# Sharath-girish/Shacira

Measured on AMD Instinct MI355X. Metric: hash-grid samples/sec fwd+bwd (16 lvl, F=2), higher is better.
Workload: dtype f32

## Files before the change

shacira_amd/csrc/api.hip:

```cpp
#include <atomic>
#include <cmath>
#include <cstdint>
#include <cstring>

#include "internal.h"

namespace shacira {

struct OptionSlot {
    const char *name;
    int Options::*field;
    int lo, hi;
    std::atomic<int> value;
};
static OptionSlot g_slots[] = {
    {"fwd_variant", &Options::fwd_variant, -1, 9, {-1}},
    {"bwd_variant", &Options::bwd_variant, -1, 1, {-1}},
    {"mlp_variant", &Options::mlp_variant, -1, 1, {-1}},
    {"bwd_compact", &Options::bwd_compact, 0, 1, {1}},
    {"bwd_selective_zero", &Options::bwd_selective_zero, 0, 1, {1}},
    {"bwd_persistent", &Options::bwd_persistent, 0, 1, {1}},
    {"bwd_fork", &Options::bwd_fork, 0, 1, {1}},
    {"bwd_run_pad", &Options::bwd_run_pad, 0, 1, {1}},
    {"bwd_item12", &Options::bwd_item12, -1, 1, {-1}},
    {"bin_acc_kib", &Options::bin_acc_kib, 0, 128, {0}},
    {"bin_batch_mib", &Options::bin_batch_mib, 1, 1 << 20, {1536}},
    {"tiled", &Options::tiled, -1, 1, {-1}},
    {"tiled_lc_fwd", &Options::tiled_lc_fwd, -1, SHACIRA_MAX_LODS, {-1}},
    {"bwd_brick", &Options::bwd_brick, -1, 1, {-1}},
    {"bwd_brick_lo", &Options::bwd_brick_lo, -1, SHACIRA_MAX_LODS, {-1}},
    {"bwd_brick_hi", &Options::bwd_brick_hi, -1, SHACIRA_MAX_LODS, {-1}},
    {"bwd_brick_fork", &Options::bwd_brick_fork, 0, 2, {2}},
    {"bwd_brick_span", &Options::bwd_brick_span, 0, 64, {0}},
    {"fwd_direct", &Options::fwd_direct, -1, 1, {-1}},
    {"bwd_ext_fork", &Options::bwd_ext_fork, 0, 1, {1}},
    {"coord_variant", &Options::coord_variant, -1, 8, {-1}},
    {"triplane_layout", &Options::triplane_layout, -1, 1, {-1}},
};
static thread_local Options tl_options;
const Options &opt() { return tl_options; }
void options_snapshot() {
    for (OptionSlot &sl : g_slots) tl_options.*(sl.field) = sl.value.load(std::memory_order_relaxed);
}
void options_resolve_item12(int value) { tl_options.bwd_item12 = value; }
static bool option_value_ok(const OptionSlot &sl, int v) {
    if (v < sl.lo || v > sl.hi) return false;
    if (!std::strcmp(sl.name, "fwd_variant")) return v == -1 || v == 0 || v == 3 || v == 6 || v == 8 || v == 9;
    if (!std::strcmp(sl.name, "coord_variant")) return v == -1 || v == 0 || v == 3 || v == 8;
    if (!std::strcmp(sl.name, "bin_acc_kib")) return v == 0 || v == 64 || v == 128;
    return true;
}

static int build_level_table(int dim, int num_lods, int feature_dim, int bw, const int32_t *res_host,
                             int64_t table_rows, LevelTable &lt) {
    if (dim != 2 && dim != 3) return SHACIRA_EINVAL;
    if (num_lods < 1 || num_lods > SHACIRA_MAX_LODS) return SHACIRA_EINVAL;
    if (feature_dim < 1) return SHACIRA_EINVAL;
    if (feature_dim % 2 == 1) return SHACIRA_EODD;
    if (bw < 1 || bw > 30) return SHACIRA_EINVAL;
    if (!res_host || table_rows < 0) return SHACIRA_EINVAL;
    std::memset(&lt, 0, sizeof(lt));
    const int32_t cs = (int32_t)std::pow(2.0, (double)bw);
    for (int l = 0; l < num_lods; ++l) {
        const int32_t r = res_host[l];
        if (r < 1) return SHACIRA_EINVAL;
        lt.res[l] = r;
        lt.hi[l] = (float)((double)r - 1.0 - 1e-5);
        lt.dense[l] = level_is_dense(dim, r, cs) ? 1 : 0;
    }
    lt.mask = (uint32_t)cs - 1u;
    lt.num_lods = num_lods;
    lt.feature_dim = feature_dim;
    lt.table_rows = table_rows;
    lt.level_begin = 0;
    lt.level_end = num_lods;
    lt.stage_flags = 0;
    return 0;
}

}

using namespace shacira;

extern "C" {

int shacira_abi_version(void) { return SHACIRA_ABI_VERSION; }

const char *shacira_strerror(int code) {
    switch (code) {
        case 0: return "success";
        case SHACIRA_EINVAL: return "shacira: invalid argument (dim/sizes/bitwidth/null pointer)";
        case SHACIRA_EDTYPE: return "shacira: unsupported scalar type or operator shape";
        case SHACIRA_EODD: return "The codebook feature dimension needs to be a multiple of 2.";
        case SHACIRA_EWORKSPACE: return "shacira: workspace too small";
        default: break;
    }
    if (code > 0) return hipGetErrorString((hipError_t)code);
    return "shacira: unknown error";
}

int shacira_set_option(const char *name, int value) {
    if (!name) return SHACIRA_EINVAL;
    for (OptionSlot &sl : g_slots) {
        if (std::strcmp(name, sl.name)) continue;
        if (!option_value_ok(sl, value)) return SHACIRA_EINVAL;
        sl.value.store(value, std::memory_order_relaxed);
        return 0;
    }
    return SHACIRA_EINVAL;
}

int shacira_get_option(const char *name) {
    if (!name) return SHACIRA_EINVAL;
    for (OptionSlot &sl : g_slots)
        if (!std::strcmp(name, sl.name)) return sl.value.load(std::memory_order_relaxed);
    return SHACIRA_EINVAL;
}

size_t shacira_hashgrid_forward_workspace_bytes(int dim, int64_t num_coords, int num_lods, int feature_dim,
                                                int codebook_bitwidth, const int32_t *resolutions_host,
                                                int64_t table_rows, int dtype) {
    options_snapshot();
    LevelTable lt;
    if (build_level_table(dim, num_lods, feature_dim, codebook_bitwidth, resolutions_host, table_rows, lt)) return 0;
    return hashgrid_forward_workspace(dim, dtype, lt, num_coords);
}

int shacira_hashgrid_forward(int dim, int64_t num_coords, int num_lods, int feature_dim, int codebook_bitwidth,
                             const int32_t *resolutions_host, const int32_t *codebook_first_idx, int64_t table_rows,
                             const float *coords, const void *codebook, int dtype, void *feats, void *workspace,
                             size_t workspace_bytes, void *stream) {
    return shacira_hashgrid_forward_planned(dim, num_coords, num_lods, feature_dim, codebook_bitwidth, resolutions_host,
                                            codebook_first_idx, table_rows, coords, codebook, dtype, feats, nullptr, 0, 0,
                                            workspace, workspace_bytes, stream);
}

size_t shacira_hashgrid_plan_bytes(int dim, int64_t num_coords, int num_lods, int feature_dim, int codebook_bitwidth,
                                   const int32_t *resolutions_host, int64_t table_rows, int dtype) {
    options_snapshot();
    LevelTable lt;
    if (build_level_table(dim, num_lods, feature_dim, codebook_bitwidth, resolutions_host, table_rows, lt)) return 0;
    if (dtype == SHACIRA_F64 || table_rows == 0 || !tiled_supported(dim, dtype, lt, num_coords)) return 0;
    return sample_plan_bytes(dim, num_coords);
}

int shacira_hashgrid_forward_planned(int dim, int64_t num_coords, int num_lods, int feature_dim, int codebook_bitwidth,
                                     const int32_t *resolutions_host, const int32_t *codebook_first_idx, int64_t table_rows,
                                     const float *coords, const void *codebook, int dtype, void *feats, void *plan,
                                     size_t plan_bytes, int plan_flags, void *workspace, size_t workspace_bytes,
                                     void *stream) {
    options_snapshot();
    LevelTable lt;
    int rc = build_level_table(dim, num_lods, feature_dim, codebook_bitwidth, resolutions_host, table_rows, lt);
    if (rc) return rc;
    if (dtype != SHACIRA_F32 && dtype != SHACIRA_F16 && dtype != SHACIRA_F64) return SHACIRA_EDTYPE;
    if (num_coords < 0) return SHACIRA_EINVAL;
    if (num_coords == 0) return 0;
    if (!codebook_first_idx || !coords || !codebook || !feats) return SHACIRA_EINVAL;
    const size_t need = hashgrid_forward_workspace(dim, dtype, lt, num_coords);
    if (need > 0 && (!workspace || workspace_bytes < need)) return SHACIRA_EWORKSPACE;
    const bool sorts = dtype != SHACIRA_F64 && table_rows > 0 && tiled_supported(dim, dtype, lt, num_coords);
    if (plan != nullptr && sorts && plan_bytes < sample_plan_bytes(dim, num_coords)) return SHACIRA_EWORKSPACE;
    if ((plan_flags & ~SHACIRA_PLAN_READY) != 0 || ((plan_flags & SHACIRA_PLAN_READY) != 0 && plan == nullptr)) return SHACIRA_EINVAL;
    return (int)hashgrid_forward_dispatch(dim, dtype, lt, codebook_first_idx, coords, codebook, feats, workspace,
                                          num_coords, (hipStream_t)stream, sorts ? plan : nullptr,
                                          (plan_flags & SHACIRA_PLAN_READY) != 0);
}

int shacira_hashgrid_debug_corners(int dim, int64_t num_coords, int num_lods, int codebook_bitwidth,
                                   const int32_t *resolutions_host, const float *coords, int32_t *corner_rows,
                                   float *corner_weights, void *stream) {
    LevelTable lt;
    int rc = build_level_table(dim, num_lods, 2, codebook_bitwidth, resolutions_host, 0, lt);
    if (rc) return rc;
    if (num_coords < 0 || num_coords * (int64_t)num_lods >= ((int64_t)1 << 31) * 256) return SHACIRA_EINVAL;
    if (num_coords > 0 && (!coords || (!corner_rows && !corner_weights))) return SHACIRA_EINVAL;
    return (int)hashgrid_debug_corners(dim, lt, coords, num_coords, corner_rows, corner_weights, (hipStream_t)stream);
}

size_t shacira_hashgrid_backward_workspace_bytes(int dim, int64_t num_coords, int num_lods, int feature_dim,
                                                 int codebook_bitwidth, const int32_t *resolutions_host,
                                                 int64_t table_rows, int dtype) {
    options_snapshot();
    LevelTable lt;
    if (build_level_table(dim, num_lods, feature_dim, codebook_bitwidth, resolutions_host, table_rows, lt)) return 0;
    return hashgrid_backward_workspace(dim, dtype, lt, num_coords);
}

int shacira_hashgrid_backward(int dim, int64_t num_coords, int num_lods, int feature_dim, int codebook_bitwidth,
                              const int32_t *resolutions_host, const int32_t *codebook_first_idx, int64_t table_rows,
                              const float *coords, const void *grad_output, int dtype, void *grad_codebook,
                              void *workspace, size_t workspace_bytes, void *stream) {
    return shacira_hashgrid_backward_levels(dim, num_coords, num_lods, feature_dim, codebook_bitwidth, resolutions_host,
                                            codebook_first_idx, table_rows, coords, grad_output, dtype, grad_codebook,
                                            0, num_lods, 0, workspace, workspace_bytes, stream);
}

static int backward_call(int dim, int64_t num_coords, int num_lods, int feature_dim, int codebook_bitwidth,
                         const int32_t *resolutions_host, const int32_t *codebook_first_idx, int64_t table_rows,
                         const float *coords, const void *grad_output, int dtype, void *grad_codebook, int level_begin,
                         int level_end, int flags, const void *plan, size_t plan_bytes, void *workspace,
                         size_t workspace_bytes, void *stream);

size_t shacira_hashgrid_backward_planned_workspace_bytes(int dim, int64_t num_coords, int num_lods, int feature_dim,
                                                         int codebook_bitwidth, const int32_t *resolutions_host,
                                                         int64_t table_rows, int dtype) {
    options_snapshot();
    LevelTable lt;
    if (build_level_table(dim, num_lods, feature_dim, codebook_bitwidth, resolutions_host, table_rows, lt)) return 0;
    LevelTable full = lt;
    const bool sorts = dtype != SHACIRA_F64 && table_rows > 0 && tiled_supported(dim, dtype, full, num_coords);
    if (!sorts) return hashgrid_backward_workspace(dim, dtype, lt, num_coords);
    return hashgrid_backward_workspace_planned(dim, dtype, lt, num_coords, true);
}

int shacira_hashgrid_backward_planned(int dim, int64_t num_coords, int num_lods, int feature_dim, int codebook_bitwidth,
                                      const int32_t *resolutions_host, const int32_t *codebook_first_idx, int64_t table_rows,
                                      const float *coords, const void *grad_output, int dtype, void *grad_codebook,
                                      const void *plan, size_t plan_bytes, void *workspace, size_t workspace_bytes,
                                      void *stream) {
    return backward_call(dim, num_coords, num_lods, feature_dim, codebook_bitwidth, resolutions_host, codebook_first_idx,
                         table_rows, coords, grad_output, dtype, grad_codebook, 0, num_lods, 0, plan, plan_bytes, workspace,
                         workspace_bytes, stream);
}

int shacira_hashgrid_backward_levels(int dim, int64_t num_coords, int num_lods, int feature_dim, int codebook_bitwidth,
                                     const int32_t *resolutions_host, const int32_t *codebook_first_idx,
                                     int64_t table_rows, const float *coords, const void *grad_output, int dtype,
                                     void *grad_codebook, int level_begin, int level_end, int flags, void *workspace,
                                     size_t workspace_bytes, void *stream) {
    return backward_call(dim, num_coords, num_lods, feature_dim, codebook_bitwidth, resolutions_host, codebook_first_idx,
                         table_rows, coords, grad_output, dtype, grad_codebook, level_begin, level_end, flags, nullptr, 0,
                         workspace, workspace_bytes, stream);
}

size_t shacira_hashgrid_coords_backward_workspace_bytes(int dim, int64_t num_coords, int num_lods, int feature_dim,
                                                        int codebook_bitwidth, const int32_t *resolutions_host,
                                                        int64_t table_rows, int dtype) {
    (void)dim; (void)num_coords; (void)num_lods; (void)feature_dim; (void)codebook_bitwidth; (void)resolutions_host;
    (void)table_rows; (void)dtype;
    return 0;
}

int shacira_hashgrid_coords_backward(int dim, int64_t num_coords, int num_lods, int feature_dim, int codebook_bitwidth,
                                     const int32_t *resolutions_host, const int32_t *codebook_first_idx, int64_t table_rows,
                                     const float *coords, const void *codebook, const void *grad_output, int dtype,
                                     float *grad_coords, const void *plan, size_t plan_bytes, void *workspace,
                                     size_t workspace_bytes, void *stream) {
    options_snapshot();
    LevelTable lt;
    int rc = build_level_table(dim, num_lods, feature_dim, codebook_bitwidth, resolutions_host, table_rows, lt);
    if (rc) return rc;
    if (dtype != SHACIRA_F32 && dtype != SHACIRA_F16 && dtype != SHACIRA_F64) return SHACIRA_EDTYPE;
    if (num_coords < 0) return SHACIRA_EINVAL;
    if (num_coords == 0) return 0;
    if (!codebook_first_idx || !coords || !codebook || !grad_output || !grad_coords) return SHACIRA_EINVAL;
    const size_t need = shacira_hashgrid_coords_backward_workspace_bytes(dim, num_coords, num_lods, feature_dim,
                                                                         codebook_bitwidth, resolutions_host, table_rows,
                                                                         dtype);
    if (need > 0 && (!workspace || workspace_bytes < need)) return SHACIRA_EWORKSPACE;
    if (plan != nullptr) {
        const bool sorts = dtype != SHACIRA_F64 && table_rows > 0 && tiled_supported(dim, dtype, lt, num_coords);
        if (!sorts) plan = nullptr;
        else if (plan_bytes < sample_plan_bytes(dim, num_coords)) return SHACIRA_EWORKSPACE;
    }
    return (int)hashgrid_coord_grad_dispatch(dim, dtype, lt, codebook_first_idx, coords, codebook, grad_output, grad_coords,
                                             num_coords, (hipStream_t)stream, plan);
}

size_t shacira_hashgrid_coords_backward2_workspace_bytes(int dim, int64_t num_coords, int num_lods, int feature_dim,
                                                         int codebook_bitwidth, const int32_t *resolutions_host,
                                                         int64_t table_rows, int dtype) {
    LevelTable lt;
    if (build_level_table(dim, num_lods, feature_dim, codebook_bitwidth, resolutions_host, table_rows, lt)) return 0;
    (void)num_coords;
    return dtype == SHACIRA_F16 ? (size_t)table_rows * (size_t)feature_dim * sizeof(float) : 0;
}

int shacira_hashgrid_coords_backward2(int dim, int64_t num_coords, int num_lods, int feature_dim, int codebook_bitwidth,
                                      const int32_t *resolutions_host, const int32_t *codebook_first_idx, int64_t table_rows,
                                      const float *coords, const void *codebook, const void *grad_output,
                                      const float *grad_grad_coords, int dtype, void *grad_grad_output, void *grad_codebook,
                                      float *grad_coords, const void *plan, size_t plan_bytes, void *workspace,
                                      size_t workspace_bytes, void *stream) {
    options_snapshot();
    LevelTable lt;
    int rc = build_level_table(dim, num_lods, feature_dim, codebook_bitwidth, resolutions_host, table_rows, lt);
    if (rc) return rc;
    if (dtype != SHACIRA_F32 && dtype != SHACIRA_F16) return SHACIRA_EDTYPE;
    if (num_coords < 0) return SHACIRA_EINVAL;
    if (!grad_grad_output && !grad_codebook && !grad_coords) return SHACIRA_EINVAL;
    if (num_coords > 0) {
        if (!codebook_first_idx || !coords || !grad_grad_coords) return SHACIRA_EINVAL;
        if (!codebook && (grad_grad_output || grad_coords)) return SHACIRA_EINVAL;
        if (!grad_output && (grad_codebook || grad_coords)) return SHACIRA_EINVAL;
        if (grad_codebook && dtype == SHACIRA_F16 && table_rows > 0) {
            const size_t need = shacira_hashgrid_coords_backward2_workspace_bytes(
                dim, num_coords, num_lods, feature_dim, codebook_bitwidth, resolutions_host, table_rows, dtype);
            if (!workspace || workspace_bytes < need) return SHACIRA_EWORKSPACE;
        }
        if (plan != nullptr) {
            const bool sorts = table_rows > 0 && tiled_supported(dim, dtype, lt, num_coords);
            if (!sorts) plan = nullptr;
            else if (plan_bytes < sample_plan_bytes(dim, num_coords)) return SHACIRA_EWORKSPACE;
        }
    }
    return (int)hashgrid_coord_grad2_dispatch(dim, dtype, lt, codebook_first_idx, coords, codebook, grad_output,
                                              grad_grad_coords, grad_grad_output, grad_codebook, grad_coords, workspace,
                                              num_coords, (hipStream_t)stream, plan);
}

static int triplane_args(int64_t num_coords, int num_lods, const int32_t *lods_host, int feature_dim, TriplaneArgs &a) {
    if (num_coords < 0 || num_coords > (int64_t)INT32_MAX) return SHACIRA_EINVAL;
    if (num_lods < 1 || num_lods > SHACIRA_TRIPLANE_MAX_LODS || !lods_host) return SHACIRA_EINVAL;
    if (feature_dim < 1 || feature_dim > SHACIRA_TRIPLANE_MAX_FDIM) return SHACIRA_EINVAL;
    std::memset(&a, 0, sizeof(a));
    a.num_lods = num_lods;
    a.fdim = feature_dim;
    for (int l = 0; l < num_lods; ++l) {
        if (lods_host[l] < 0 || lods_host[l] > SHACIRA_TRIPLANE_MAX_LOD) return SHACIRA_EINVAL;
        a.side[l] = (1 << lods_host[l]) + 1;
    }
    return 0;
}

static int triplane_pointers(int num_lods, const float *const *host, TriplaneArgs &a, bool grad) {
    if (!host) return SHACIRA_EINVAL;
    for (int q = 0; q < 3 * num_lods; ++q) {
        if (!host[q]) return SHACIRA_EINVAL;
        if (grad) a.grad[q] = const_cast<float *>(host[q]);
        else a.plane[q] = host[q];
    }
    return 0;
}

size_t shacira_triplane_forward_workspace_bytes(int64_t num_coords, int num_lods, const int32_t *lods_host,
                                                int feature_dim, int multiscale_sum) {
    options_snapshot();
    TriplaneArgs a;
    if (triplane_args(num_coords, num_lods, lods_host, feature_dim, a)) return 0;
    return triplane_forward_workspace(a, num_coords);
}

int shacira_triplane_forward(int64_t num_coords, int num_lods, const int32_t *lods_host, int feature_dim,
                             const float *coords, const float *const *planes_host, int multiscale_sum, float *feats,
                             void *workspace, size_t workspace_bytes, void *stream) {
    options_snapshot();
    TriplaneArgs a;
    if (int rc = triplane_args(num_coords, num_lods, lods_host, feature_dim, a)) return rc;
    if (multiscale_sum != 0 && multiscale_sum != 1) return SHACIRA_EINVAL;
    if (num_coords == 0) return 0;
    if (!coords || !feats) return SHACIRA_EINVAL;
    if (int rc = triplane_pointers(num_lods, planes_host, a, false)) return rc;
    const size_t need = triplane_forward_workspace(a, num_coords);
    if (need > 0 && (!workspace || workspace_bytes < need)) return SHACIRA_EWORKSPACE;
    return (int)triplane_forward_dispatch(a, coords, multiscale_sum, feats, workspace, num_coords, (hipStream_t)stream);
}

size_t shacira_triplane_backward_workspace_bytes(int64_t num_coords, int num_lods, const int32_t *lods_host,
                                                 int feature_dim, int multiscale_sum, int flags) {
    TriplaneArgs a;
    if (triplane_args(num_coords, num_lods, lods_host, feature_dim, a)) return 0;
    if ((flags & SHACIRA_TRIPLANE_GRAD_PLANES) == 0) return 0;
    return triplane_backward_workspace(a, multiscale_sum, num_coords);
}

int shacira_triplane_backward(int64_t num_coords, int num_lods, const int32_t *lods_host, int feature_dim,
                              const float *coords, const float *const *planes_host, const float *grad_output,
                              int multiscale_sum, int flags, float *const *grad_planes_host, float *grad_coords,
                              void *workspace, size_t workspace_bytes, void *stream) {
    TriplaneArgs a;
    if (int rc = triplane_args(num_coords, num_lods, lods_host, feature_dim, a)) return rc;
    if (multiscale_sum != 0 && multiscale_sum != 1) return SHACIRA_EINVAL;
    if (flags <= 0 || (flags & ~(SHACIRA_TRIPLANE_GRAD_PLANES | SHACIRA_TRIPLANE_GRAD_COORDS)) != 0) return SHACIRA_EINVAL;
    const bool planes = (flags & SHACIRA_TRIPLANE_GRAD_PLANES) != 0;
    const bool want_coords = (flags & SHACIRA_TRIPLANE_GRAD_COORDS) != 0;
    if (planes)
        if (int rc = triplane_pointers(num_lods, const_cast<const float *const *>(grad_planes_host), a, true)) return rc;
    if (num_coords > 0) {
        if (!coords || !grad_output) return SHACIRA_EINVAL;
        if (want_coords) {
            if (!grad_coords) return SHACIRA_EINVAL;
            if (int rc = triplane_pointers(num_lods, planes_host, a, false)) return rc;
        }
    }
    const size_t need = planes ? triplane_backward_workspace(a, multiscale_sum, num_coords) : 0;
    if (need > 0 && (!workspace || workspace_bytes < need)) return SHACIRA_EWORKSPACE;
    return (int)triplane_backward_dispatch(a, coords, grad_output, multiscale_sum, planes,
                                           want_coords ? grad_coords : nullptr, workspace, num_coords,
                                           (hipStream_t)stream);
}

static int octree_args(int64_t num_coords, int num_levels, const int32_t *levels_host, int feature_dim, OctreeArgs &a) {
    if (num_coords < 0 || num_coords > (int64_t)INT32_MAX) return SHACIRA_EINVAL;
    if (num_levels < 1 || num_levels > SHACIRA_OCTREE_MAX_LEVELS || !levels_host) return SHACIRA_EINVAL;
    if (feature_dim < 1 || feature_dim > SHACIRA_OCTREE_MAX_FDIM) return SHACIRA_EINVAL;
    std::memset(&a, 0, sizeof(a));
    a.num_levels = num_levels;
    a.fdim = feature_dim;
    for (int l = 0; l < num_levels; ++l) {
        if (levels_host[l] < 0 || levels_host[l] > SHACIRA_OCTREE_MAX_LEVEL) return SHACIRA_EINVAL;
        a.level[l] = levels_host[l];
    }
    return 0;
}

static int octree_rows(const int64_t *rows_host, OctreeArgs &a) {
    if (!rows_host) return SHACIRA_EINVAL;
    for (int l = 0; l < a.num_levels; ++l) {
        const int64_t side = ((int64_t)1 << a.level[l]) + 1;
        if (rows_host[l] < 0 || rows_host[l] > side * side * side) return SHACIRA_EINVAL;
        a.rows[l] = rows_host[l];
    }
    return 0;
}

static int octree_index(const void *const *corner_index_host, const void *const *occupancy_host, OctreeArgs &a) {
    if (!corner_index_host || !occupancy_host) return SHACIRA_EINVAL;
    for (int l = 0; l < a.num_levels; ++l) {
        if (!corner_index_host[l] || !occupancy_host[l]) return SHACIRA_EINVAL;
        a.corner[l] = static_cast<const uint2 *>(corner_index_host[l]);
        a.occ[l] = static_cast<const uint32_t *>(occupancy_host[l]);
    }
    return 0;
}

static int octree_tables(const float *const *tables_host, OctreeArgs &a) {
    if (!tables_host) return SHACIRA_EINVAL;
    for (int l = 0; l < a.num_levels; ++l) {
        if (!tables_host[l]) return SHACIRA_EINVAL;
        a.table[l] = tables_host[l];
    }
    return 0;
}

size_t shacira_octree_forward_workspace_bytes(int64_t num_coords, int num_levels, const int32_t *levels_host,
                                              int feature_dim, int multiscale_sum) {
    return 0;
}

int shacira_octree_forward(int64_t num_coords, int num_levels, const int32_t *levels_host, int feature_dim,
                           const float *coords, const float *const *tables_host, const int64_t *rows_host,
                           const void *const *corner_index_host, const void *const *occupancy_host, int multiscale_sum,
                           float *feats, void *workspace, size_t workspace_bytes, void *stream) {
    OctreeArgs a;
    if (int rc = octree_args(num_coords, num_levels, levels_host, feature_dim, a)) return rc;
    if (multiscale_sum != 0 && multiscale_sum != 1) return SHACIRA_EINVAL;
    if (int rc = octree_rows(rows_host, a)) return rc;
    if (num_coords == 0) return 0;
    if (!coords || !feats) return SHACIRA_EINVAL;
    if (int rc = octree_tables(tables_host, a)) return rc;
    if (int rc = octree_index(corner_index_host, occupancy_host, a)) return rc;
    return (int)octree_forward_dispatch(a, coords, multiscale_sum, feats, num_coords, (hipStream_t)stream);
}

size_t shacira_octree_backward_workspace_bytes(int64_t num_coords, int num_levels, const int32_t *levels_host,
                                               int feature_dim, int multiscale_sum, int flags) {
    OctreeArgs a;
    if (octree_args(num_coords, num_levels, levels_host, feature_dim, a)) return 0;
    if ((flags & SHACIRA_OCTREE_GRAD_FEATURES) == 0) return 0;
    return octree_backward_workspace(a, multiscale_sum, num_coords);
}

int shacira_octree_backward(int64_t num_coords, int num_levels, const int32_t *levels_host, int feature_dim,
// ... 800 lines not shown
```

shacira_amd/csrc/hashgrid_fwd.hip:

```cpp
#include <mutex>

#include "hashgrid_rows.h"
#include "internal.h"

namespace shacira {

static bool use_staged(int dim, const LevelTable &lt, int64_t n);
static bool use_lds_tables(int dim, int esz, const LevelTable &lt, int64_t n);

template <typename T, int F> __device__ __forceinline__ void store_row(T *p, const float (&v)[F]) {
    if constexpr (sizeof(T) == 4 && F == 2) {
        *reinterpret_cast<float2 *>(p) = make_float2(v[0], v[1]);
    } else if constexpr (sizeof(T) == 4 && F == 4) {
        *reinterpret_cast<float4 *>(p) = make_float4(v[0], v[1], v[2], v[3]);
    } else if constexpr (sizeof(T) == 2 && F == 2) {
        *reinterpret_cast<__half2 *>(p) = __floats2half2_rn(Scalar<__half>::rounded_fp32(v[0]), Scalar<__half>::rounded_fp32(v[1]));
    } else {
#pragma unroll
        for (int j = 0; j < F; ++j) Scalar<T>::store(p + j, v[j]);
    }
}

template <int DIM, typename T, int F>
__global__ __launch_bounds__(256) void hashgrid_fwd_kernel(LevelTable lt, const int32_t *__restrict__ first_idx,
// ... 530 lines not shown
        int32_t p[DIM];
#pragma unroll
        for (int a = 0; a < DIM; ++a) axis_transform(t[a], res, hi, p[a], f[u][a], g[u][a]);
        const uint32_t ux = (uint32_t)p[0] + (uint32_t)dx;
#pragma unroll
        for (int q = 0; q < NH; ++q) {
            const int dy = (DIM == 3) ? (q >> 1) : q;
            const int dz = (DIM == 3) ? (q & 1) : 0;
            const uint32_t uy = (uint32_t)p[1] + dy;
            uint32_t row;
            if (dense) {
                row = ux + uy * r;
                if constexpr (DIM == 3) row += ((uint32_t)p[2] + dz) * r * r;
            } else {
                row = ux ^ (uy * kPrimeY);
                if constexpr (DIM == 3) row ^= ((uint32_t)p[2] + dz) * kPrimeZ;
                row &= lt.mask;
            }
            const int64_t grow = base + (int64_t)row;
            gather_row<T, F>(table, grow, live[u] && (uint64_t)grow < (uint64_t)lt.table_rows, v[u][q]);
        }
    }
#pragma unroll
    for (int u = 0; u < U; ++u) {
        float pv[NH][F];
#pragma unroll
        for (int q = 0; q < NH; ++q)
#pragma unroll
            for (int j = 0; j < F; ++j)
                pv[q][j] = __builtin_bit_cast(
                    float, __builtin_amdgcn_mov_dpp(__builtin_bit_cast(int, v[u][q][j]), 0xB1, 0xF, 0xF, true));
        if (dx == 0 && live[u]) {
            float acc[F];
#pragma unroll
            for (int k = 0; k < 2 * NH; ++k) {
                const int kx = k / NH, q = k % NH;
                const int dy = (DIM == 3) ? (q >> 1) : q;
                const int dz = (DIM == 3) ? (q & 1) : 0;
                float w = (kx ? f[u][0] : g[u][0]) * (dy ? f[u][1] : g[u][1]);
                if constexpr (DIM == 3) w = w * (dz ? f[u][2] : g[u][2]);
#pragma unroll
                for (int j = 0; j < F; ++j) {
                    const float tv = kx ? pv[q][j] : v[u][q][j];
                    acc[j] = (k == 0) ? tv * w : fmaf(tv, w, acc[j]);
                }
            }
            T *dstT = feats + (int64_t)lvl * level_stride + idx[u] * sample_stride;
            if constexpr (sizeof(T) == 4 && F == 2) {
                typedef float f32x2 __attribute__((ext_vector_type(2)));
                f32x2 o = {acc[0], acc[1]};
                *reinterpret_cast<f32x2 *>(dstT) = o;
            } else {
                store_row<T, F>(dstT, acc);
            }
        }
    }
}

template <typename T, int F>
__global__ __launch_bounds__(256) void untranspose_feats_kernel(const T *__restrict__ src, T *__restrict__ dst,
                                                                int64_t N, int L) {
    struct alignas(sizeof(T) * F) Piece { T v[F]; };
    extern __shared__ __align__(16) unsigned char s_raw_t[];
    Piece *s_tile = reinterpret_cast<Piece *>(s_raw_t);
    const int pitch = L + 1;
    const int64_t s0 = (int64_t)blockIdx.x * 256;
    const int ns = (int)((N - s0 < 256) ? (N - s0) : 256);
    const Piece *in = reinterpret_cast<const Piece *>(src);
    for (int l = 0; l < L; ++l)
        if ((int)threadIdx.x < ns) s_tile[threadIdx.x * pitch + l] = in[(int64_t)l * N + s0 + threadIdx.x];
    __syncthreads();
    const int total = ns * L;
    Piece *out = reinterpret_cast<Piece *>(dst) + s0 * L;
    for (int e = threadIdx.x; e < total; e += 256) {
        const int sm = e / L, l = e - sm * L;
        out[e] = s_tile[sm * pitch + l];
    }
}

template <typename T> static size_t staged_bytes(const LevelTable &lt, int64_t n) {
    return ((size_t)n * lt.num_lods * lt.feature_dim * sizeof(T) + 255) / 256 * 256;
}

template <int DIM, typename T, int F>
static hipError_t launch_fwd(const LevelTable &lt, const int32_t *first_idx, const float *coords, const void *table,
                             void *feats, void *workspace, int64_t num_coords, hipStream_t stream) {
    const int variant = opt().fwd_variant;
    if constexpr (F > 0) {
        if (use_lds_tables(DIM, (int)sizeof(T), lt, num_coords) && ((size_t)lt.num_lods * F * sizeof(T)) % 16 == 0 &&
            (reinterpret_cast<uintptr_t>(feats) & 15u) == 0) {
            LdsFwdPlan plan;
            make_lds_fwd_plan(DIM, lt, sizeof(T), plan);
            static PerDeviceOnce once;
            hipError_t e = once.run([]() -> hipError_t {
                return hipFuncSetAttribute(reinterpret_cast<const void *>(&hashgrid_fwd_lds_kernel<DIM, T, F>),
                                           hipFuncAttributeMaxDynamicSharedMemorySize, (int)kLdsFwdBytes);
            });
            if (e != hipSuccess) return e;
            uint32_t bpg = 256u / (uint32_t)plan.ngroups;
            const uint64_t spw = (uint64_t)kLdsFwdThreads / (uint64_t)plan.P;
            const uint64_t need = ((uint64_t)num_coords + spw - 1) / spw;
            if (bpg > need) bpg = (uint32_t)need;
            if (bpg < 1) bpg = 1;
            hipLaunchKernelGGL((hashgrid_fwd_lds_kernel<DIM, T, F>), dim3(bpg, (uint32_t)plan.ngroups), dim3(kLdsFwdThreads),
                               kLdsFwdBytes, stream, lt, plan, first_idx, coords, static_cast<const T *>(table),
                               static_cast<T *>(feats), num_coords);
            return hipGetLastError();
        }
        if (use_staged(DIM, lt, num_coords) && workspace) {
            const uint32_t tiles = (uint32_t)((num_coords + 128 * kLevelPairU - 1) / (128 * kLevelPairU));
            const uint32_t grid_v6 = 8u * (uint32_t)(((uint64_t)lt.num_lods * tiles + 7) / 8);
            hipError_t e;
            const int d_opt = opt().fwd_direct;
            if (d_opt == 1 || (d_opt < 0 && num_coords <= SHACIRA_FWD_DIRECT_MAX)) {
                hipLaunchKernelGGL((hashgrid_fwd_level_pair_kernel<DIM, T, F>), dim3(grid_v6), dim3(256), 0, stream, lt,
                                   first_idx, coords, static_cast<const T *>(table), static_cast<T *>(feats), num_coords, tiles,
                                   (int64_t)F, (int64_t)lt.num_lods * F);
                return hipGetLastError();
            }
            hipLaunchKernelGGL((hashgrid_fwd_level_pair_kernel<DIM, T, F>), dim3(grid_v6),
                               dim3(256), 0, stream, lt, first_idx, coords, static_cast<const T *>(table),
                               static_cast<T *>(workspace), num_coords, tiles, num_coords * F, (int64_t)F);
            e = hipGetLastError();
            if (e != hipSuccess) return e;
            const size_t shmem = (size_t)256 * (lt.num_lods + 1) * F * sizeof(T);
            static PerDeviceOnce once;
            e = once.run([]() -> hipError_t {
                return hipFuncSetAttribute(reinterpret_cast<const void *>(&untranspose_feats_kernel<T, F>),
                                           hipFuncAttributeMaxDynamicSharedMemorySize, 140 * 1024);
            });
            if (e != hipSuccess) return e;
            hipLaunchKernelGGL((untranspose_feats_kernel<T, F>), dim3((uint32_t)((num_coords + 255) / 256)), dim3(256),
                               shmem, stream, static_cast<const T *>(workspace), static_cast<T *>(feats), num_coords,
                               lt.num_lods);
            return hipGetLastError();
        }
        if (variant == 3 || variant < 0) {
            const uint32_t blocks = (uint32_t)((num_coords + 127) / 128);
            const int LFP = (lt.num_lods * F + 3) / 4 * 4 + 4;
            const size_t shmem = (size_t)128 * LFP * sizeof(float);
            if (shmem <= 64 * 1024) {
                hipLaunchKernelGGL((hashgrid_fwd_pair_kernel<DIM, T, F>), dim3(blocks), dim3(256), shmem, stream, lt,
                                   first_idx, coords, static_cast<const T *>(table), static_cast<T *>(feats),
                                   num_coords);
                return hipGetLastError();
            }
        }
    }
    const int64_t L = lt.num_lods;
    const int64_t max_samples = ((int64_t)1 << 31) / L - 1;
    for (int64_t s0 = 0; s0 < num_coords; s0 += max_samples) {
        const int64_t ns = (num_coords - s0 < max_samples) ? (num_coords - s0) : max_samples;
        const uint32_t items = (uint32_t)(ns * L);
        const uint32_t blocks = (items + 255u) / 256u;
        hipLaunchKernelGGL((hashgrid_fwd_kernel<DIM, T, F>), dim3(blocks), dim3(256), 0, stream, lt, first_idx, coords,
                           static_cast<const T *>(table), static_cast<T *>(feats), s0, items);
        hipError_t e = hipGetLastError();
        if (e != hipSuccess) return e;
    }
    return hipSuccess;
}

template <int DIM, typename T>
static hipError_t dispatch_f(const LevelTable &lt, const int32_t *first_idx, const float *coords, const void *table,
                             void *feats, void *ws, int64_t n, hipStream_t s) {
    switch (lt.feature_dim) {
        case 2: return launch_fwd<DIM, T, 2>(lt, first_idx, coords, table, feats, ws, n, s);
        case 4: return launch_fwd<DIM, T, 4>(lt, first_idx, coords, table, feats, ws, n, s);
        default: return launch_fwd<DIM, T, 0>(lt, first_idx, coords, table, feats, ws, n, s);
    }
}

static bool use_lds_tables(int dim, int esz, const LevelTable &lt, int64_t n) {
    const int v = opt().fwd_variant;
    if (lt.feature_dim != 2 && lt.feature_dim != 4) return false;
    if (v >= 0 && v != 9) return false;
    if (n < 1 || n >= ((int64_t)1 << 31)) return false;
    LdsFwdPlan p;
    if (!make_lds_fwd_plan(dim, lt, (size_t)esz, p)) return false;
    return v == 9 || n >= 4096;
}

static bool use_staged(int dim, const LevelTable &lt, int64_t n) {
    const int v = opt().fwd_variant;
    if (lt.feature_dim != 2 && lt.feature_dim != 4) return false;
    if (v == 6) return true;
    return v < 0 && dim == 3 && n >= 8192;
}

template <int DIM, typename T, int F>
static hipError_t launch_levels_staged(const LevelTable &lt, const int32_t *first_idx, const float *coords,
                                       const void *table, void *staged, int64_t n, hipStream_t s) {
    const uint32_t nl = (uint32_t)(lt.level_end - lt.level_begin);
    const uint32_t tiles = (uint32_t)((n + 128 * kLevelPairU - 1) / (128 * kLevelPairU));
    hipLaunchKernelGGL((hashgrid_fwd_level_pair_kernel<DIM, T, F, true>),
                       dim3(8u * (uint32_t)(((uint64_t)nl * tiles + 7) / 8)), dim3(256), 0, s,
                       lt, first_idx, coords, static_cast<const T *>(table), static_cast<T *>(staged), n, tiles, n * F,
                       (int64_t)F);
    return hipGetLastError();
}

hipError_t hashgrid_forward_levels_staged(int dim, int dtype, const LevelTable &lt, const int32_t *first_idx,
                                          const float *coords, const void *table, void *staged, int64_t n,
                                          hipStream_t s) {
    const int F = lt.feature_dim;
    if (F != 2 && F != 4) return hipErrorInvalidValue;
    if (dim == 3 && dtype == SHACIRA_F32)
        return F == 2 ? launch_levels_staged<3, float, 2>(lt, first_idx, coords, table, staged, n, s)
                      : launch_levels_staged<3, float, 4>(lt, first_idx, coords, table, staged, n, s);
    if (dim == 3)
        return F == 2 ? launch_levels_staged<3, __half, 2>(lt, first_idx, coords, table, staged, n, s)
                      : launch_levels_staged<3, __half, 4>(lt, first_idx, coords, table, staged, n, s);
    if (dtype == SHACIRA_F32)
        return F == 2 ? launch_levels_staged<2, float, 2>(lt, first_idx, coords, table, staged, n, s)
                      : launch_levels_staged<2, float, 4>(lt, first_idx, coords, table, staged, n, s);
    return F == 2 ? launch_levels_staged<2, __half, 2>(lt, first_idx, coords, table, staged, n, s)
                  : launch_levels_staged<2, __half, 4>(lt, first_idx, coords, table, staged, n, s);
}

template <int DIM, typename T, int F>
static hipError_t launch_rows(const LevelTable &lt, const int32_t *first_idx, const float *sorted4,
                              const void *table, const void *staged, void *feats, int64_t n, int lc, hipStream_t s) {
    const uint32_t row_bytes = (uint32_t)(lt.num_lods * F * sizeof(T));
    const size_t shmem = (size_t)128 * ((row_bytes + 15u) / 16u * 16u + 16u);
    static PerDeviceOnce once;
    const hipError_t oe = once.run([]() -> hipError_t {
        return hipFuncSetAttribute(reinterpret_cast<const void *>(&hashgrid_fwd_rows_kernel<DIM, T, F>),
                                   hipFuncAttributeMaxDynamicSharedMemorySize, 140 * 1024);
    });
    if (oe != hipSuccess) return oe;
    const uint32_t blocks = ((uint32_t)((n + 127) / 128) + 7u) & ~7u;
    hipLaunchKernelGGL((hashgrid_fwd_rows_kernel<DIM, T, F>), dim3(blocks), dim3(256), shmem, s, lt,
                       first_idx, reinterpret_cast<const float4 *>(sorted4), static_cast<const T *>(table),
                       static_cast<const T *>(staged), static_cast<T *>(feats), n, lc, 1u);
    return hipGetLastError();
}

hipError_t hashgrid_forward_rows(int dim, int dtype, const LevelTable &lt, const int32_t *first_idx, const float *sorted4,
                                 const void *table, const void *staged, void *feats, int64_t n, int lc, hipStream_t s) {
    const int F = lt.feature_dim;
    if (F != 2 && F != 4) return hipErrorInvalidValue;
    if (dim == 3 && dtype == SHACIRA_F32)
        return F == 2 ? launch_rows<3, float, 2>(lt, first_idx, sorted4, table, staged, feats, n, lc, s)
                      : launch_rows<3, float, 4>(lt, first_idx, sorted4, table, staged, feats, n, lc, s);
    if (dim == 3)
        return F == 2 ? launch_rows<3, __half, 2>(lt, first_idx, sorted4, table, staged, feats, n, lc, s)
                      : launch_rows<3, __half, 4>(lt, first_idx, sorted4, table, staged, feats, n, lc, s);
    if (dtype == SHACIRA_F32)
        return F == 2 ? launch_rows<2, float, 2>(lt, first_idx, sorted4, table, staged, feats, n, lc, s)
                      : launch_rows<2, float, 4>(lt, first_idx, sorted4, table, staged, feats, n, lc, s);
    return F == 2 ? launch_rows<2, __half, 2>(lt, first_idx, sorted4, table, staged, feats, n, lc, s)
                  : launch_rows<2, __half, 4>(lt, first_idx, sorted4, table, staged, feats, n, lc, s);
}

template <int DIM>
__global__ __launch_bounds__(256) void debug_corners_kernel(LevelTable lt, const float *__restrict__ coords, int64_t N,
                                                            int32_t *__restrict__ idx, float *__restrict__ w) {
    constexpr int NC = 1 << DIM;
    const int64_t e = (int64_t)blockIdx.x * 256 + threadIdx.x;
    const int L = lt.num_lods;
    if (e >= N * L) return;
    const int64_t i = e / L;
    const int l = (int)(e - i * L);
    double t[DIM];
#pragma unroll
    for (int a = 0; a < DIM; ++a) t[a] = axis_unit(coords[i * DIM + a]);
    Corners<DIM> c;
    compute_corners<DIM>(t, lt.res[l], lt.hi[l], lt.dense[l] != 0, lt.mask, c);
#pragma unroll
    for (int k = 0; k < NC; ++k) {
        if (idx) idx[e * NC + k] = (int32_t)c.row[k];
        if (w) w[e * NC + k] = c.w[k];
    }
}

hipError_t hashgrid_debug_corners(int dim, const LevelTable &lt, const float *coords, int64_t n, int32_t *idx, float *w,
                                  hipStream_t s) {
    const int64_t items = n * lt.num_lods;
    if (items <= 0) return hipSuccess;
    const uint32_t blocks = (uint32_t)((items + 255) / 256);
    if (dim == 3)
        hipLaunchKernelGGL(debug_corners_kernel<3>, dim3(blocks), dim3(256), 0, s, lt, coords, n, idx, w);
    else
        hipLaunchKernelGGL(debug_corners_kernel<2>, dim3(blocks), dim3(256), 0, s, lt, coords, n, idx, w);
    return hipGetLastError();
}

template <int DIM>
static hipError_t launch_fwd_f64(const LevelTable &lt, const int32_t *first_idx, const float *coords, const void *table,
                                 void *feats, int64_t num_coords, hipStream_t stream) {
    const int64_t L = lt.num_lods;
    const int64_t max_samples = ((int64_t)1 << 31) / L - 1;
    for (int64_t s0 = 0; s0 < num_coords; s0 += max_samples) {
        const int64_t ns = (num_coords - s0 < max_samples) ? (num_coords - s0) : max_samples;
        const uint32_t items = (uint32_t)(ns * L);
        hipLaunchKernelGGL((hashgrid_fwd_kernel<DIM, double, 0>), dim3((items + 255u) / 256u), dim3(256), 0, stream, lt,
                           first_idx, coords, static_cast<const double *>(table), static_cast<double *>(feats), s0, items);
        hipError_t e = hipGetLastError();
        if (e != hipSuccess) return e;
    }
    return hipSuccess;
}

size_t hashgrid_forward_workspace(int dim, int dtype, const LevelTable &lt, int64_t n) {
    if (dtype == SHACIRA_F64) return 0;
    if (tiled_supported(dim, dtype, lt, n)) return tiled_forward_workspace(dim, dtype, lt, n);
    if (lt.feature_dim != 2 && lt.feature_dim != 4) return 0;
    if (use_lds_tables(dim, dtype == SHACIRA_F32 ? 4 : 2, lt, n)) return 0;
    size_t b = ((size_t)n * lt.num_lods * lt.feature_dim * (dtype == SHACIRA_F32 ? 4 : 2) + 255) / 256 * 256;
    return b;
}

hipError_t hashgrid_forward_dispatch(int dim, int dtype, const LevelTable &lt, const int32_t *first_idx,
                                     const float *coords, const void *table, void *feats, void *ws, int64_t n,
                                     hipStream_t s, void *plan, bool plan_ready) {
    if (lt.table_rows == 0) {
        const size_t bytes = (size_t)n * lt.num_lods * lt.feature_dim * (dtype == SHACIRA_F64 ? 8 : dtype == SHACIRA_F32 ? 4 : 2);
        return zero_fill_async(static_cast<float *>(feats), (int64_t)(bytes / 4), s);
    }
    if (dtype == SHACIRA_F64)
        return dim == 3 ? launch_fwd_f64<3>(lt, first_idx, coords, table, feats, n, s)
                        : launch_fwd_f64<2>(lt, first_idx, coords, table, feats, n, s);
    if (tiled_supported(dim, dtype, lt, n)) return tiled_forward(dim, dtype, lt, first_idx, coords, table, feats, ws, n, s, plan, plan_ready);
    if (dim == 3) {
        return dtype == SHACIRA_F32 ? dispatch_f<3, float>(lt, first_idx, coords, table, feats, ws, n, s)
                                    : dispatch_f<3, __half>(lt, first_idx, coords, table, feats, ws, n, s);
    }
    return dtype == SHACIRA_F32 ? dispatch_f<2, float>(lt, first_idx, coords, table, feats, ws, n, s)
                                : dispatch_f<2, __half>(lt, first_idx, coords, table, feats, ws, n, s);
}

}
```

shacira_amd/csrc/hashgrid_tiled.hip:

```cpp
#include <cmath>
#include <mutex>

#include "internal.h"

namespace shacira {

constexpr int kTargetPerBlock = 352;
#ifndef SHACIRA_SORT_TILE
#define SHACIRA_SORT_TILE 4096
#endif
constexpr int kSortTileS = SHACIRA_SORT_TILE;
constexpr int kSortThreadsS = 1024;
constexpr int kMaxBlocksS = 4096;
constexpr int kMaxAxisBlocks = 64;
constexpr uint32_t kCtxMagic = 0x53484354u;

constexpr int kMaxCoarse = 256;
constexpr int kMaxSortTiles = 512;

struct TilePlan {
    int32_t nb[3];
    uint32_t num_blocks;
    int32_t lc;
    uint32_t coarse_shift, num_coarse;
    uint32_t ptiles, chunks_per_tile;
};

struct TileCtx {
    uint32_t *header;
    float4 *sorted4;
    uint32_t *block_start;
    uint32_t *cnt;
    float4 *inter4;
    uint32_t *gcursor;
    uint32_t *cbase;
};

static inline size_t up256(size_t v) { return (v + 255) / 256 * 256; }

__host__ __device__ inline uint32_t axis_block(float c, int nb) {
    const float u = (c + 1.0f) * (0.5f * (float)nb);
    if (!(u < (float)nb)) return (uint32_t)(nb - 1);
    if (!(u >= 0.0f)) return 0u;
    return (uint32_t)(int)u;
}

template <int DIM> __device__ __forceinline__ uint32_t block_key(const float (&c)[DIM], const TilePlan &tp) {
    uint32_t k = axis_block(c[0], tp.nb[0]) + (uint32_t)tp.nb[0] * axis_block(c[1], tp.nb[1]);
    if constexpr (DIM == 3) k += (uint32_t)(tp.nb[0] * tp.nb[1]) * axis_block(c[2], tp.nb[2]);
    return k;
}

static void make_sort_plan(int dim, int64_t n, TilePlan &tp) {
    const double want = (double)n / kTargetPerBlock;
    tp.nb[0] = tp.nb[1] = tp.nb[2] = 1;
    auto clampi = [](double v) { int q = (int)(v + 0.5); return q < 1 ? 1 : (q > kMaxAxisBlocks ? kMaxAxisBlocks : q); };
    if (dim == 3) {
        int m = clampi(std::cbrt(want / 2.0));
        if (m > 12) m = 12;
        tp.nb[0] = tp.nb[1] = m;
        int z = clampi(want / ((double)m * m));
        while ((int64_t)m * m * z > kMaxBlocksS) --z;
        tp.nb[2] = z;
    } else {
        const int m = clampi(std::sqrt(want / 2.0));
        tp.nb[0] = m;
        int y = clampi(want / m);
        while ((int64_t)m * y > kMaxBlocksS) --y;
        tp.nb[1] = y;
    }
    tp.num_blocks = (uint32_t)(tp.nb[0] * tp.nb[1] * tp.nb[2]);
    tp.lc = 0;
    tp.coarse_shift = 0;
    while (((tp.num_blocks + (1u << tp.coarse_shift) - 1) >> tp.coarse_shift) > (uint32_t)kMaxCoarse) ++tp.coarse_shift;
    tp.num_coarse = (tp.num_blocks + (1u << tp.coarse_shift) - 1) >> tp.coarse_shift;
    const int64_t chunks = (n + kSortTileS - 1) / kSortTileS;
    tp.chunks_per_tile = (uint32_t)((chunks + kMaxSortTiles - 1) / kMaxSortTiles);
    if (tp.chunks_per_tile < 1) tp.chunks_per_tile = 1;
    tp.ptiles = (uint32_t)((chunks + tp.chunks_per_tile - 1) / tp.chunks_per_tile);
}

static void make_tile_plan(int dim, const LevelTable &lt, int64_t n, TilePlan &tp) {
    make_sort_plan(dim, n, tp);
    int lc = 0;
    while (lc < lt.num_lods) {
        double cells = 1.0;
        for (int a = 0; a < dim; ++a) cells *= (double)lt.res[lc];
        if (dim == 3 && cells > 32.0 * (double)n) break;
        ++lc;
    }
    const int lc_opt = opt().tiled_lc_fwd;
    if (lc_opt >= 0 && lc_opt <= lt.num_lods) lc = lc_opt;
    tp.lc = lc;
}

static size_t carve_plan(int64_t n, void *buf, TileCtx &c) {
    size_t off = 0;
    auto take = [&](size_t b) { size_t o = off; off = up256(off + b); return o; };
    const size_t o_hdr = take(256);
    const size_t o_sorted = take((size_t)n * sizeof(float4));
    const size_t o_bs = take((size_t)(kMaxBlocksS + 1) * 4);
    unsigned char *p = static_cast<unsigned char *>(buf);
    if (p) {
        c.header = reinterpret_cast<uint32_t *>(p + o_hdr);
        c.sorted4 = reinterpret_cast<float4 *>(p + o_sorted);
        c.block_start = reinterpret_cast<uint32_t *>(p + o_bs);
    }
    return off;
}
static size_t carve_scratch(int dim, int64_t n, void *buf, TileCtx &c) {
    (void)dim;
    size_t off = 0;
    auto take = [&](size_t b) { size_t o = off; off = up256(off + b); return o; };
    const size_t o_cnt = take((size_t)kMaxSortTiles * kMaxCoarse * 4);
    const size_t o_inter = take((size_t)n * sizeof(float4));
    const size_t o_cb = take((size_t)(kMaxCoarse + 1) * 4);
    const size_t o_gc = take((size_t)2 * kMaxBlocksS * 4);
    unsigned char *p = static_cast<unsigned char *>(buf);
    if (p) {
        c.cnt = reinterpret_cast<uint32_t *>(p + o_cnt);
        c.inter4 = reinterpret_cast<float4 *>(p + o_inter);
        c.cbase = reinterpret_cast<uint32_t *>(p + o_cb);
        c.gcursor = reinterpret_cast<uint32_t *>(p + o_gc);
    }
    return off;
}
static size_t plan_bytes_of(int64_t n) {
    TileCtx c{};
    return carve_plan(n, nullptr, c);
}
static size_t scratch_bytes_of(int dim, int64_t n) {
    TileCtx c{};
    return carve_scratch(dim, n, nullptr, c);
}

template <int DIM>
__device__ __forceinline__ void load_chunk_coords(const float *__restrict__ coords, int64_t s0, int64_t N,
                                                  float (&c)[kSortTileS / kSortThreadsS][DIM]) {
    constexpr int U = kSortTileS / kSortThreadsS;
#pragma unroll
    for (int u = 0; u < U; ++u) {
        const int64_t i = s0 + u * kSortThreadsS + threadIdx.x;
        const int64_t ic = i < N ? i : N - 1;
#pragma unroll
        for (int a = 0; a < DIM; ++a) c[u][a] = coords[ic * DIM + a];
    }
}

constexpr int kLocalR = 8;
constexpr uint32_t kLocalCap = kLocalR * kSortThreadsS;

template <int DIM>
__global__ __launch_bounds__(kSortThreadsS) void psort_count_kernel(TilePlan tp, const float *__restrict__ coords,
                                                                    int64_t N, uint32_t *__restrict__ cnt,
                                                                    uint32_t *__restrict__ gcursor) {
    __shared__ uint32_t s_hist[kMaxCoarse];
    if (threadIdx.x < kMaxCoarse) s_hist[threadIdx.x] = 0;
    if (blockIdx.x == 0)
        for (uint32_t k = threadIdx.x; k < 2u * kMaxBlocksS; k += kSortThreadsS) gcursor[k] = 0u;
    __syncthreads();
    constexpr int U = kSortTileS / kSortThreadsS;
    for (uint32_t ch = 0; ch < tp.chunks_per_tile; ++ch) {
        const int64_t s0 = ((int64_t)blockIdx.x * tp.chunks_per_tile + ch) * kSortTileS;
        if (s0 >= N) break;
        float c[U][DIM];
        load_chunk_coords<DIM>(coords, s0, N, c);
#pragma unroll
        for (int u = 0; u < U; ++u)
            if (s0 + u * kSortThreadsS + threadIdx.x < N) atomicAdd(&s_hist[block_key<DIM>(c[u], tp) >> tp.coarse_shift], 1u);
    }
    __syncthreads();
    if (threadIdx.x < kMaxCoarse) cnt[(size_t)threadIdx.x * kMaxSortTiles + blockIdx.x] = s_hist[threadIdx.x];
}

template <int DIM>
__global__ __launch_bounds__(kSortThreadsS) void psort_partition_kernel(TilePlan tp, const float *__restrict__ coords,
                                                                        int64_t N, const uint32_t *__restrict__ cnt,
                                                                        uint32_t *__restrict__ cbase,
                                                                        uint32_t *__restrict__ gcursor,
                                                                        float4 *__restrict__ inter4) {
    __shared__ uint32_t s_cursor[kMaxCoarse], s_tot[kMaxCoarse], s_before[kMaxCoarse];
    __shared__ uint32_t s_wave[kMaxCoarse / 64];
    const uint32_t lane = threadIdx.x & 63, wave = threadIdx.x >> 6;
    constexpr int U = kSortTileS / kSortThreadsS;
    float c0[U][DIM];
    const int64_t first_s0 = (int64_t)blockIdx.x * tp.chunks_per_tile * kSortTileS;
    load_chunk_coords<DIM>(coords, first_s0 < N ? first_s0 : 0, N, c0);
    typedef uint32_t u32x4 __attribute__((ext_vector_type(4)));
    constexpr int kWaves = kSortThreadsS / 64, kBinsPerWave = kMaxCoarse / kWaves;
    const bool wide = tp.ptiles > 256u;
#ifndef SHACIRA_SORT_RB
#define SHACIRA_SORT_RB 8
#endif
    constexpr int RB = SHACIRA_SORT_RB;
#pragma unroll 1
    for (int g = 0; g < kBinsPerWave; g += RB) {
        u32x4 v[RB], w[RB];
#pragma unroll
        for (int k = 0; k < RB; ++k) {
            const u32x4 *row = reinterpret_cast<const u32x4 *>(cnt + (size_t)(wave * kBinsPerWave + g + k) * kMaxSortTiles);
            v[k] = row[lane];
            w[k] = wide ? row[64 + lane] : u32x4{0u, 0u, 0u, 0u};
        }
#pragma unroll
        for (int k = 0; k < RB; ++k) {
            uint32_t tot = 0, before = 0;
#pragma unroll
            for (int e = 0; e < 4; ++e) {
                const uint32_t t0 = lane * 4u + (uint32_t)e, t1 = 256u + t0;
                const uint32_t a = t0 < tp.ptiles ? v[k][e] : 0u, b2 = t1 < tp.ptiles ? w[k][e] : 0u;
                tot += a + b2;
                before += (t0 < blockIdx.x ? a : 0u) + (t1 < blockIdx.x ? b2 : 0u);
            }
#pragma unroll
            for (int off = 32; off > 0; off >>= 1) {
                tot += __shfl_xor(tot, off, 64);
                before += __shfl_xor(before, off, 64);
            }
            if (lane == 0) {
                s_tot[wave * kBinsPerWave + g + k] = tot;
                s_before[wave * kBinsPerWave + g + k] = before;
            }
        }
    }
    __syncthreads();
    const bool owner = threadIdx.x < kMaxCoarse;
    uint32_t tot = 0;
    if (owner) {
        tot = s_tot[threadIdx.x];
        uint32_t incl = tot;
#pragma unroll
        for (int off = 1; off < 64; off <<= 1) {
            const uint32_t nbr = __shfl_up(incl, off, 64);
            if (lane >= (uint32_t)off) incl += nbr;
        }
        if (lane == 63) s_wave[wave] = incl;
        s_cursor[threadIdx.x] = incl - tot;
    }
    __syncthreads();
    uint32_t base = 0;
    if (owner) {
        for (uint32_t wv = 0; wv < wave; ++wv) base += s_wave[wv];
        base += s_cursor[threadIdx.x];
        if (blockIdx.x == 0) {
            cbase[threadIdx.x] = base;
            if (threadIdx.x == kMaxCoarse - 1) cbase[kMaxCoarse] = base + tot;
        }
    }
    __shared__ uint32_t s_over_any;
    __shared__ uint32_t s_blk[kMaxBlocksS];
    if (threadIdx.x == 0) s_over_any = 0u;
    __syncthreads();
    if (owner) {
        s_cursor[threadIdx.x] = base + s_before[threadIdx.x];
        if (tot > kLocalCap) s_over_any = 1u;
        s_tot[threadIdx.x] = tot > kLocalCap ? 1u : 0u;
    }
    __syncthreads();
    const bool over_any = s_over_any != 0u;
    if (over_any) {
        for (uint32_t k = threadIdx.x; k < tp.num_blocks; k += kSortThreadsS) s_blk[k] = 0u;
        __syncthreads();
    }
    for (uint32_t ch = 0; ch < tp.chunks_per_tile; ++ch) {
        const int64_t s0 = first_s0 + (int64_t)ch * kSortTileS;
        if (s0 >= N) break;
        float c[U][DIM];
        if (ch == 0) {
#pragma unroll
            for (int u = 0; u < U; ++u)
#pragma unroll
                for (int a = 0; a < DIM; ++a) c[u][a] = c0[u][a];
        } else {
            load_chunk_coords<DIM>(coords, s0, N, c);
        }
        uint32_t pos[U];
#pragma unroll
        for (int u = 0; u < U; ++u) {
            const int64_t i = s0 + u * kSortThreadsS + threadIdx.x;
            const uint32_t key = block_key<DIM>(c[u], tp);
            pos[u] = (i < N) ? atomicAdd(&s_cursor[key >> tp.coarse_shift], 1u) : 0xFFFFFFFFu;
            if (over_any && i < N && s_tot[key >> tp.coarse_shift]) atomicAdd(&s_blk[key], 1u);
        }
#pragma unroll
        for (int u = 0; u < U; ++u) {
            const int64_t i = s0 + u * kSortThreadsS + threadIdx.x;
            if (pos[u] != 0xFFFFFFFFu) {
                typedef float f32x4 __attribute__((ext_vector_type(4)));
                const f32x4 rec = {c[u][0], c[u][1], DIM == 3 ? c[u][DIM - 1] : 0.0f, __uint_as_float((uint32_t)i)};
#ifdef SHACIRA_SORT_NT
                __builtin_nontemporal_store(rec, reinterpret_cast<f32x4 *>(inter4 + pos[u]));
#else
                *reinterpret_cast<f32x4 *>(inter4 + pos[u]) = rec;
#endif
            }
        }
    }
    if (over_any) {
        __syncthreads();
        uint32_t *gcount = gcursor + kMaxBlocksS;
        for (uint32_t k = threadIdx.x; k < tp.num_blocks; k += kSortThreadsS)
            if (s_blk[k]) atomicAdd(&gcount[k], s_blk[k]);
    }
}

__device__ __forceinline__ uint32_t wave_rank_add(uint32_t *counters, uint32_t j, bool live, uint32_t lane) {
    const uint64_t lm = __ballot(live);
    if (lm == 0ull) return 0u;
    const uint32_t leader = (uint32_t)__builtin_ctzll(lm);
    const uint32_t j0 = (uint32_t)__shfl((int)j, (int)leader, 64);
    const uint64_t same = __ballot(live && j == j0);
    if (same == lm) {
        uint32_t b = 0;
        if (lane == leader) b = atomicAdd(&counters[j0], (uint32_t)__popcll(lm));
        b = (uint32_t)__shfl((int)b, (int)leader, 64);
        return b + (uint32_t)__popcll(lm & ((1ull << lane) - 1ull));
    }
    return live ? atomicAdd(&counters[j], 1u) : 0u;
}

template <int DIM>
__global__ __launch_bounds__(kSortThreadsS) void psort_local_kernel(TilePlan tp, const float4 *__restrict__ inter4,
                                                                    const uint32_t *__restrict__ cbase,
                                                                    const uint32_t *__restrict__ gcount,
                                                                    uint32_t *__restrict__ gcursor,
                                                                    float4 *__restrict__ sorted4,
                                                                    uint32_t *__restrict__ block_start,
                                                                    uint32_t *__restrict__ header, uint32_t n) {
    constexpr int kBpc = kMaxBlocksS / kMaxCoarse;
    constexpr int R = kLocalR;
    uint32_t bin, lo, hi, c_lo, c_hi;
    const bool first = blockIdx.x < tp.num_coarse;
    if (first) {
        bin = blockIdx.x;
        lo = cbase[bin];
        hi = cbase[bin + 1];
        c_lo = lo;
        c_hi = (lo + kLocalCap < hi) ? lo + kLocalCap : hi;
    } else {
        const uint32_t p0 = (blockIdx.x - tp.num_coarse) * kLocalCap;
        if (p0 >= n) return;
        __shared__ uint32_t s_le;
        if (threadIdx.x == 0) s_le = 0u;
        __syncthreads();
        uint32_t c = (threadIdx.x < tp.num_coarse && cbase[threadIdx.x] <= p0) ? 1u : 0u;
        if (threadIdx.x < kMaxCoarse) {
#pragma unroll
            for (int off = 32; off > 0; off >>= 1) c += __shfl_xor(c, off, 64);
            if ((threadIdx.x & 63u) == 0u && c) atomicAdd(&s_le, c);
        }
        __syncthreads();
        bin = s_le - 1u;
        lo = cbase[bin];
        hi = cbase[bin + 1];
        c_lo = (lo + kLocalCap > p0) ? lo + kLocalCap : p0;
        c_hi = (p0 + kLocalCap < hi) ? p0 + kLocalCap : hi;
        if (c_lo >= c_hi) return;
    }
    const uint32_t key0 = bin << tp.coarse_shift;
    const uint32_t bpc = 1u << tp.coarse_shift;
    const uint32_t lane = threadIdx.x & 63;
    auto key_of = [&](const float4 &r) {
        float cc[DIM];
        cc[0] = r.x;
        cc[1] = r.y;
        if constexpr (DIM == 3) cc[2] = r.z;
        return block_key<DIM>(cc, tp) - key0;
    };
    if (blockIdx.x == 0 && threadIdx.x == 0) {
        header[0] = kCtxMagic;
        header[1] = tp.num_blocks;
        header[2] = n;
    }
    if (first && hi - lo <= kLocalCap) {
#ifndef SHACIRA_SORT_SUB
#define SHACIRA_SORT_SUB 2
#endif
        constexpr int kSubBits = SHACIRA_SORT_SUB;
        constexpr int kSub = 1 << (kSubBits * DIM);
        constexpr int kKeys = kBpc * kSub;
        __shared__ uint32_t s_tot8[kKeys], s_wtot[16];
        uint32_t *s_off8 = s_tot8;
        for (uint32_t k = threadIdx.x; k < (uint32_t)kKeys; k += kSortThreadsS) s_tot8[k] = 0;
        __syncthreads();
        auto sub_of = [&](const float4 &r) -> uint32_t {
            if constexpr (kSub == 1) return 0u;
            uint32_t sb = 0;
            const float cc[3] = {r.x, r.y, r.z};
#pragma unroll
            for (int a = 0; a < DIM; ++a) {
                const float u = (cc[a] + 1.0f) * (0.5f * (float)tp.nb[a]);
                const float fr = u - floorf(u);
                uint32_t q = (uint32_t)(int)(fr * (float)(1 << kSubBits));
                q = q < (1u << kSubBits) ? q : (1u << kSubBits) - 1u;
                sb |= q << (a * kSubBits);
            }
            return sb;
        };
        float4 r[R];
        uint32_t j[R], rk[R];
#pragma unroll
        for (int u = 0; u < R; ++u) {
            const uint32_t p = lo + (uint32_t)u * kSortThreadsS + threadIdx.x;
            r[u] = inter4[p < hi ? p : (hi > 0u ? hi - 1u : 0u)];
        }
#pragma unroll
        for (int u = 0; u < R; ++u) {
            const bool live = lo + (uint32_t)u * kSortThreadsS + threadIdx.x < hi;
            j[u] = live ? key_of(r[u]) * (uint32_t)kSub + sub_of(r[u]) : 0u;
            rk[u] = wave_rank_add(s_tot8, j[u], live, lane);
        }
        __syncthreads();
        {
            constexpr int KPT = (kKeys + kSortThreadsS - 1) / kSortThreadsS;
            uint32_t cnt[KPT], sum = 0;
#pragma unroll
            for (int q = 0; q < KPT; ++q) {
                const uint32_t k = threadIdx.x * KPT + q;
                cnt[q] = k < (uint32_t)kKeys ? s_tot8[k] : 0u;
                sum += cnt[q];
            }
            uint32_t incl = sum;
#pragma unroll
            for (int off = 1; off < 64; off <<= 1) {
                const uint32_t nbr = __shfl_up(incl, off, 64);
                if (lane >= (uint32_t)off) incl += nbr;
            }
            if (lane == 63) s_wtot[threadIdx.x >> 6] = incl;
            __syncthreads();
            uint32_t run = incl - sum;
            for (uint32_t w = 0; w < (threadIdx.x >> 6); ++w) run += s_wtot[w];
#pragma unroll
            for (int q = 0; q < KPT; ++q) {
                const uint32_t k = threadIdx.x * KPT + q;
                if (k < (uint32_t)kKeys) s_off8[k] = run;
                run += cnt[q];
            }
        }
        __syncthreads();
        if (threadIdx.x < bpc && key0 + threadIdx.x < tp.num_blocks) block_start[key0 + threadIdx.x] = lo + s_off8[threadIdx.x * kSub];
        if (bin + 1u == tp.num_coarse && threadIdx.x == 0) block_start[tp.num_blocks] = hi;
#pragma unroll
        for (int u = 0; u < R; ++u)
            if (lo + (uint32_t)u * kSortThreadsS + threadIdx.x < hi) sorted4[lo + s_off8[j[u]] + rk[u]] = r[u];
        return;
    }
    __shared__ uint32_t s_off[kBpc + 1], s_cnt[kBpc], s_base[kBpc];
    if (threadIdx.x == 0) {
        uint32_t run = 0;
        for (uint32_t b = 0; b < bpc; ++b) {
            s_off[b] = run;
            run += (key0 + b < tp.num_blocks) ? gcount[key0 + b] : 0u;
        }
        s_off[bpc] = run;
    }
    if (threadIdx.x < kBpc) s_cnt[threadIdx.x] = 0;
    __syncthreads();
    if (first) {
        if (threadIdx.x < bpc && key0 + threadIdx.x < tp.num_blocks) block_start[key0 + threadIdx.x] = lo + s_off[threadIdx.x];
        if (bin + 1u == tp.num_coarse && threadIdx.x == 0) block_start[tp.num_blocks] = hi;
    }
    float4 r[R];
    uint32_t j[R], rk[R];
#pragma unroll
    for (int u = 0; u < R; ++u) {
        const uint32_t p = c_lo + (uint32_t)u * kSortThreadsS + threadIdx.x;
        r[u] = inter4[p < c_hi ? p : c_hi - 1u];
    }
#pragma unroll
    for (int u = 0; u < R; ++u) {
        const bool live = c_lo + (uint32_t)u * kSortThreadsS + threadIdx.x < c_hi;
        j[u] = live ? key_of(r[u]) : 0u;
        rk[u] = wave_rank_add(s_cnt, j[u], live, lane);
    }
    __syncthreads();
    if (threadIdx.x < bpc) s_base[threadIdx.x] = s_cnt[threadIdx.x] ? atomicAdd(&gcursor[key0 + threadIdx.x], s_cnt[threadIdx.x]) : 0u;
    __syncthreads();
#pragma unroll
    for (int u = 0; u < R; ++u)
        if (c_lo + (uint32_t)u * kSortThreadsS + threadIdx.x < c_hi) sorted4[lo + s_off[j[u]] + s_base[j[u]] + rk[u]] = r[u];
}

bool tiled_supported(int dim, int dtype, const LevelTable &lt, int64_t n) {
    const int t_opt = opt().tiled;
    if (t_opt == 0) return false;
    const int v = opt().fwd_variant;
    if (v >= 0 && v != 8) return false;
    if (lt.feature_dim != 2 && lt.feature_dim != 4) return false;
    if (n < 1 || n >= ((int64_t)1 << 31)) return false;
    if (t_opt == 1 || v == 8) return true;
    const size_t table_bytes = (size_t)lt.table_rows * lt.feature_dim * (dtype == SHACIRA_F32 ? 4 : 2);
    if (table_bytes < ((size_t)8 << 20)) return false;
    if (dim == 2) return n >= ((int64_t)3 << 16);
    return n >= (lt.feature_dim == 4 ? (int64_t)80 << 10 : (int64_t)1 << 18);
}

static size_t staged_bytes(int dtype, const LevelTable &lt, int64_t n) {
    return up256((size_t)n * lt.num_lods * lt.feature_dim * (dtype == SHACIRA_F32 ? 4 : 2));
}

#define SHACIRA_CHECK_LAUNCH()                 \
    do {                                       \
        hipError_t e_ = hipGetLastError();     \
        if (e_ != hipSuccess) return e_;       \
    } while (0)

size_t sample_plan_bytes(int dim, int64_t n) {
    (void)dim;
    return n > 0 ? plan_bytes_of(n) : 0;
}
size_t sample_plan_scratch_bytes(int dim, int64_t n) { return n > 0 ? scratch_bytes_of(dim, n) : 0; }

hipError_t sample_plan_build(int dim, const float *coords, int64_t n, void *plan, void *scratch, hipStream_t s) {
    TilePlan tp;
    make_sort_plan(dim, n, tp);
    TileCtx c{};
    carve_plan(n, plan, c);
    carve_scratch(dim, n, scratch, c);
    const uint32_t chunks = tp.num_coarse + (uint32_t)((n + kLocalCap - 1) / kLocalCap);
    uint32_t *gcount = c.gcursor + kMaxBlocksS;
#define SHACIRA_SORT_LAUNCHES(D)                                                                                          \
    hipLaunchKernelGGL(psort_count_kernel<D>, dim3(tp.ptiles), dim3(kSortThreadsS), 0, s, tp, coords, n, c.cnt, c.gcursor);  \
    SHACIRA_CHECK_LAUNCH();                                                                                                  \
    hipLaunchKernelGGL(psort_partition_kernel<D>, dim3(tp.ptiles), dim3(kSortThreadsS), 0, s, tp, coords, n, c.cnt, c.cbase, \
                       c.gcursor, c.inter4);                                                                                 \
    SHACIRA_CHECK_LAUNCH();                                                                                                  \
    hipLaunchKernelGGL(psort_local_kernel<D>, dim3(chunks), dim3(kSortThreadsS), 0, s, tp, c.inter4, c.cbase, gcount,        \
                       c.gcursor, c.sorted4, c.block_start, c.header, (uint32_t)n);
    if (dim == 3) {
        SHACIRA_SORT_LAUNCHES(3)
    } else {
        SHACIRA_SORT_LAUNCHES(2)
    }
#undef SHACIRA_SORT_LAUNCHES
    SHACIRA_CHECK_LAUNCH();
    return hipSuccess;
}

void sample_plan_grid(int dim, int64_t n, SortedBatch &out) {
    TilePlan tp;
    make_sort_plan(dim, n, tp);
    out.sorted4 = nullptr;
    out.block_start = nullptr;
    out.num_blocks = tp.num_blocks;
    for (int a = 0; a < 3; ++a) out.nb[a] = tp.nb[a];
}

void sample_plan_view(int dim, int64_t n, const void *plan, SortedBatch &out) {
    TilePlan tp;
    make_sort_plan(dim, n, tp);
    TileCtx c{};
    carve_plan(n, const_cast<void *>(plan), c);
    out.sorted4 = c.sorted4;
    out.block_start = c.block_start;
    out.num_blocks = tp.num_blocks;
    for (int a = 0; a < 3; ++a) out.nb[a] = tp.nb[a];
}

size_t tiled_forward_workspace(int dim, int dtype, const LevelTable &lt, int64_t n) {
    return staged_bytes(dtype, lt, n) + scratch_bytes_of(dim, n) + plan_bytes_of(n);
}

hipError_t tiled_forward(int dim, int dtype, const LevelTable &lt, const int32_t *first_idx, const float *coords,
                         const void *table, void *feats, void *workspace, int64_t n, hipStream_t s, void *plan,
                         bool plan_ready) {
    TilePlan tp;
    make_tile_plan(dim, lt, n, tp);
    unsigned char *ws = static_cast<unsigned char *>(workspace);
    void *staged = ws;
    unsigned char *scratch = ws + staged_bytes(dtype, lt, n);
    if (plan == nullptr) plan = scratch + scratch_bytes_of(dim, n);
    if (!plan_ready) {
        hipError_t e = sample_plan_build(dim, coords, n, plan, scratch, s);
        if (e != hipSuccess) return e;
    }
    TileCtx ctx{};
    carve_plan(n, plan, ctx);
    const int L = lt.num_lods;
    if (tp.lc < L) {
        LevelTable fine = lt;
        fine.level_begin = tp.lc;
        fine.level_end = L;
        hipError_t e = hashgrid_forward_levels_staged(dim, dtype, fine, first_idx, reinterpret_cast<const float *>(ctx.sorted4),
                                                      table, staged, n, s);
        if (e != hipSuccess) return e;
    }
    return hashgrid_forward_rows(dim, dtype, lt, first_idx, reinterpret_cast<const float *>(ctx.sorted4), table, staged,
                                 feats, n, tp.lc, s);
}

}
```

shacira_amd/csrc/internal.h:

```cpp
#pragma once

#include <atomic>
#include <mutex>

#include "hashgrid_device.h"

namespace shacira {

constexpr int kMaxDevices = 64;
struct PerDeviceOnce {
    std::once_flag flag[kMaxDevices];
    hipError_t err[kMaxDevices] = {};
    template <typename Fn> hipError_t run(Fn &&fn) {
        int dev = 0;
        hipError_t e = hipGetDevice(&dev);
        if (e != hipSuccess) return e;
        if (dev < 0 || dev >= kMaxDevices) return hipErrorInvalidDevice;
        std::call_once(flag[dev], [&] { err[dev] = fn(); });
        return err[dev];
    }
};

size_t hashgrid_forward_workspace(int dim, int dtype, const LevelTable &lt, int64_t n);
hipError_t hashgrid_forward_dispatch(int dim, int dtype, const LevelTable &lt, const int32_t *first_idx,
                                     const float *coords, const void *table, void *feats, void *workspace, int64_t n,
                                     hipStream_t s, void *plan = nullptr, bool plan_ready = false);
hipError_t hashgrid_forward_levels_staged(int dim, int dtype, const LevelTable &lt, const int32_t *first_idx,
                                          const float *coords, const void *table, void *staged, int64_t n,
                                          hipStream_t s);
hipError_t hashgrid_forward_rows(int dim, int dtype, const LevelTable &lt, const int32_t *first_idx, const float *sorted4,
                                 const void *table, const void *staged, void *feats, int64_t n, int lc, hipStream_t s);
bool tiled_supported(int dim, int dtype, const LevelTable &lt, int64_t n);
size_t tiled_forward_workspace(int dim, int dtype, const LevelTable &lt, int64_t n);
hipError_t tiled_forward(int dim, int dtype, const LevelTable &lt, const int32_t *first_idx, const float *coords,
                         const void *table, void *feats, void *workspace, int64_t n, hipStream_t s, void *plan = nullptr,
                         bool plan_ready = false);
struct SortedBatch {
    const float4 *sorted4;
    const uint32_t *block_start;
    uint32_t num_blocks;
    int32_t nb[3];
};
size_t sample_plan_bytes(int dim, int64_t n);
size_t sample_plan_scratch_bytes(int dim, int64_t n);
hipError_t sample_plan_build(int dim, const float *coords, int64_t n, void *plan, void *scratch, hipStream_t s);
void sample_plan_view(int dim, int64_t n, const void *plan, SortedBatch &out);
void sample_plan_grid(int dim, int64_t n, SortedBatch &out);
hipError_t hashgrid_debug_corners(int dim, const LevelTable &lt, const float *coords, int64_t n, int32_t *idx, float *w,
                                  hipStream_t s);
hipError_t hashgrid_coord_grad_dispatch(int dim, int dtype, const LevelTable &lt, const int32_t *first_idx,
                                        const float *coords, const void *table, const void *grad_out,
                                        float *grad_coords, int64_t n, hipStream_t s, const void *plan);
hipError_t hashgrid_coord_grad2_dispatch(int dim, int dtype, const LevelTable &lt, const int32_t *first_idx,
                                         const float *coords, const void *table, const void *grad_out, const float *vv,
                                         void *ggo, void *grad_table, float *grad_coords, void *workspace, int64_t n,
                                         hipStream_t s, const void *plan);
hipError_t zero_fill_async(float *p, int64_t n, hipStream_t s);
size_t hashgrid_backward_workspace(int dim, int dtype, const LevelTable &lt, int64_t n);
size_t hashgrid_backward_workspace_planned(int dim, int dtype, const LevelTable &lt, int64_t n, bool grad_aligned);
hipError_t hashgrid_backward_dispatch(int dim, int dtype, const LevelTable &lt, const int32_t *first_idx,
                                      const float *coords, const void *grad_out, void *grad_table, void *workspace,
                                      size_t workspace_bytes, int64_t n, hipStream_t s, const void *plan = nullptr);

struct TriplaneArgs {
    const float *plane[3 * SHACIRA_TRIPLANE_MAX_LODS];
    float *grad[3 * SHACIRA_TRIPLANE_MAX_LODS];
    int64_t hwc_off[3 * SHACIRA_TRIPLANE_MAX_LODS];
    int32_t side[SHACIRA_TRIPLANE_MAX_LODS];
    int32_t num_lods;
    int32_t fdim;
};
struct TriBwdPlan {
    int32_t nb, nbins;
    int32_t sort_side;
    int32_t cells;
    int32_t sum;
    int32_t win[SHACIRA_TRIPLANE_MAX_LODS];
};
constexpr int kTriDefaultHwc = 1;
size_t triplane_forward_workspace(const TriplaneArgs &a, int64_t n);
hipError_t triplane_forward_dispatch(TriplaneArgs a, const float *coords, int sum, float *feats, void *workspace,
                                     int64_t n, hipStream_t s);
void triplane_backward_plan(const TriplaneArgs &a, int sum, TriBwdPlan &bp);
size_t triplane_backward_workspace(const TriplaneArgs &a, int sum, int64_t n);
hipError_t triplane_backward_dispatch(const TriplaneArgs &a, const float *coords, const float *grad_out, int sum,
                                      bool planes, float *grad_coords, void *workspace, int64_t n, hipStream_t s);

struct OctreeArgs {
    const float *table[SHACIRA_OCTREE_MAX_LEVELS];
    float *grad[SHACIRA_OCTREE_MAX_LEVELS];
    const uint2 *corner[SHACIRA_OCTREE_MAX_LEVELS];
    const uint32_t *occ[SHACIRA_OCTREE_MAX_LEVELS];
    int64_t rows[SHACIRA_OCTREE_MAX_LEVELS];
    int32_t level[SHACIRA_OCTREE_MAX_LEVELS];
    int32_t num_levels;
    int32_t fdim;
};
struct OctBwdPlan {
    int32_t fine;
    int32_t cells_log2;
    int32_t nb, nbins;
    int32_t sum;
    int32_t wside[SHACIRA_OCTREE_MAX_LEVELS];
    int32_t woff[SHACIRA_OCTREE_MAX_LEVELS];
    int32_t wtotal;
};
void octree_backward_plan(const OctreeArgs &a, int sum, OctBwdPlan &bp);
size_t octree_backward_workspace(const OctreeArgs &a, int sum, int64_t n);
hipError_t octree_forward_dispatch(const OctreeArgs &a, const float *coords, int sum, float *feats, int64_t n,
                                   hipStream_t s);
hipError_t octree_backward_dispatch(const OctreeArgs &a, const float *coords, const float *grad_out, int sum,
                                    bool features, float *grad_coords, void *workspace, int64_t n, hipStream_t s);

size_t mesh_sdf_workspace(int64_t n, int64_t t);
hipError_t mesh_sdf_dispatch(int64_t n, int64_t t, const float *points, const float *tris, float *sdf, void *workspace,
                             hipStream_t s);
size_t mesh_closest_workspace(int64_t n, int64_t t);
hipError_t mesh_closest_dispatch(int64_t n, int64_t t, const float *points, const float *tris, bool is_signed, float *dist,
                                 float *hit, int32_t *tidx, void *workspace, hipStream_t s);

size_t mesh_voxelize_workspace(int64_t t);
hipError_t mesh_voxelize_dispatch(int64_t t, const float *tris, int level, float margin, uint32_t *words, uint8_t *grid,
                                  void *workspace, hipStream_t s);

int64_t ssim_tiles(int64_t H, int64_t W);
size_t ssim_workspace(int64_t H, int64_t W, int C, bool backward);
hipError_t ssim_forward_dispatch(int64_t H, int64_t W, int cin, int C, const float *x, const float *y, float data_range,
                                 double *value, float *map, void *workspace, hipStream_t s);
hipError_t ssim_backward_dispatch(int64_t H, int64_t W, int cin, int C, const float *x, const float *y, float data_range,
                                  const float *grad, float *grad_x, void *workspace, hipStream_t s);

hipError_t posenc_forward_dispatch(int64_t n, int d, int F, int I, int P, const float *coords, int64_t cstride,
                                   const float *prefix, int64_t pstride, const float *bands, float *out, int64_t ostride,
                                   hipStream_t s);
hipError_t posenc_backward_dispatch(int64_t n, int d, int F, int I, int P, const float *row, int64_t rstride,
                                    const float *grad_out, int64_t gstride, const float *bands, float *grad_coords,
                                    hipStream_t s);
hipError_t posenc_backward2_dispatch(int64_t n, int d, int F, int I, int P, const float *gg, const float *row, int64_t rstride,
                                     const float *grad_out, int64_t gstride, const float *bands, float *grad_row,
                                     float *grad_grad, hipStream_t s);

hipError_t raygen_dispatch(const float *cams, int num_views, int width, int height, const int32_t *view_idx,
                           const int32_t *pixel_idx, const float *jitter, int64_t n, const uint8_t *images, int channels,
                           bool bg_black, float *origins, float *dirs, float *rgb, uint8_t *mask, hipStream_t s);

hipError_t find_depth_bound_launch(int64_t P, int64_t K, const float *query, const int32_t *curr, const int32_t *pack_end,
                                   const float *depth, int32_t *out, hipStream_t s);
hipError_t sphere_trace_step_launch(int64_t P, int64_t K, int64_t num_active, bool first, const int32_t *active_in,
                                    const float *sdf, const float *origins, const float *dirs, const float *depth,
                                    const int32_t *pack_end, const int32_t *pidx, float step_size, float min_dis,
                                    float dist_max, float *t, float *dist, float *dist_prev, int32_t *curr, float *x,
                                    uint8_t *active, uint8_t *hit, int32_t *active_out, float *coords_out,
                                    int32_t *pidx_out, int32_t *count_out, int32_t *count_next, hipStream_t s);

struct DecodeArgs {
    const float *latent, *div, *matrix, *colscale, *shift;
    float clampw;
    float *decoded;
    const float *grad_decoded;
    float *grad_latent, *grad_matrix, *grad_colscale, *grad_shift;
    double *partials;
    int64_t rows;
    const float *uniforms;
    float temperature;
    int diff_sampling;
    const float *temperature_dev;
};
struct MultiArgs {
    const float *latent, *alpha, *div, *scale, *dft, *shift, *uniforms, *grad_decoded;
    float *decoded, *grad_latent, *grad_alpha, *grad_scale, *grad_shift;
    double *partials;
    int64_t rows;
    int K, straight_through, diff_sampling;
    float temperature, clampw;
};
struct EntropyArgs {
    const float *latent, *noise, *params, *grad_total;
    int num_layers;
    float *total_bits, *grad_latent, *grad_params;
    double *partials;
    int64_t rows;
};
struct LatentMlpArgs {
    int num_layers;
    const int32_t *widths;
    const float *latent, *uniforms, *div, *params;
    float temperature;
    int diff_sampling, act, final_act;
    float clampw;
    float *decoded;
    const float *grad_decoded;
    float *grad_latent, *grad_params;
    double *partials;
    int64_t rows;
};
bool latent_mlp_supported(int num_layers, const int32_t *widths);
size_t latent_mlp_workspace_bytes(int num_layers, const int32_t *widths);
hipError_t latent_mlp_dispatch(bool bwd, const LatentMlpArgs &a, hipStream_t s);

size_t latent_workspace_bytes();
bool latent_decode_supported(int ld, int f);
hipError_t latent_decode_dispatch(bool bwd, int ld, int f, int levels, const int64_t *offsets, const DecodeArgs &a,
                                  hipStream_t s);
bool latent_multi_supported(int ld, int f, int K);
hipError_t latent_multi_dispatch(bool bwd, int ld, int f, bool dft, const MultiArgs &a, hipStream_t s);
bool entropy_supported(int ld);
hipError_t entropy_dispatch(bool bwd, int ld, const EntropyArgs &a, hipStream_t s);

bool symbols_supported(int ld);
hipError_t symbol_range_launch(const float *latent, int64_t rows, int ld, int32_t *minmax, hipStream_t s);
hipError_t symbol_histogram_launch(const float *latent, int64_t rows, int ld, const int32_t *minmax, int nbins,
                                   uint64_t *counts, hipStream_t s);
size_t rc_encode_bound(int64_t n);
int rc_encode(const int32_t *sym, int64_t n, const uint32_t *freq, int nsym, uint8_t *out, size_t cap, size_t *len);
int rc_decode(const uint8_t *in, size_t len, const uint32_t *freq, int nsym, int64_t n, int32_t *sym);
bool rans_steps_ok(int steps);
size_t rans_encode_bound(int64_t n, int steps);
int rans_encode(const int32_t *sym, int64_t n, const uint32_t *freq, int nsym, int steps, uint8_t *out, size_t cap,
                size_t *len);
int rans_decode(const uint8_t *in, size_t len, const uint32_t *freq, int nsym, int64_t n, int steps, int32_t *sym);
int rans_device_args_ok(int64_t rows, int ld, const int32_t *nbins, int cdf_stride, int steps, const int64_t *payload,
                        const int64_t *words, size_t bytes);
hipError_t rans_encode_launch(const float *latent, int64_t rows, int ld, const int32_t *lo, const int32_t *nbins,
                              const uint32_t *cdf, int cdf_stride, int steps, uint32_t *counts, uint32_t *states,
                              uint16_t *slots, hipStream_t s);
hipError_t rans_pack_launch(int64_t rows, int ld, const int32_t *nbins, int steps, const uint32_t *counts,
                            const uint32_t *states, const uint16_t *slots, const int64_t *block_start,
                            const int64_t *payload, const int64_t *words, uint8_t *out, hipStream_t s);
hipError_t rans_decode_launch(const uint8_t *data, int64_t rows, int ld, const int32_t *lo, const int32_t *nbins,
                              const int64_t *payload, const int64_t *words, const uint32_t *cdf, int cdf_stride,
                              const int64_t *block_start, int steps, float *out, int32_t *error, hipStream_t s);

hipError_t pack_integrate_launch(bool bwd, int64_t R, int C, const float *feats, const float *tau,
                                 const int64_t *pack_start, float *ray_feats, float *weights, const float *g_ray,
                                 const float *g_w, float *g_feats, float *g_tau, hipStream_t s);
hipError_t pack_sum_launch(bool broadcast, int64_t R, int C, const float *in, const int64_t *pack_start, float *out,
                           hipStream_t s);
hipError_t raymarch_ray_launch(bool emit, int64_t num_rays, int ns, const float *origins, const float *dirs,
                               float dist_min, float dist_max, const float *lin, const float *jitter,
                               const uint8_t *occ, int level, int32_t *counts, const int64_t *offsets, int64_t *ridx,
                               float *samples, float *depth, float *deltas, uint8_t *boundary, int64_t capacity,
                               hipStream_t s);
hipError_t raytrace_dense_launch(bool emit, int64_t num_rays, const float *origins, const float *dirs,
                                 const uint8_t *occ, int level, int32_t *counts, const int64_t *offsets, int32_t *ridx,
                                 int32_t *pidx, float *depth, hipStream_t s);

hipError_t stream_probe_launch(int kind, const void *a, void *b, size_t bytes, uint32_t *sink, hipStream_t s);

hipError_t adam_step_launch(float *p, float *g, float *m, float *v, int64_t n, float lr, float b1, float b2, float eps,
                            float wd, int step, const int32_t *step_dev, int zero_grad, hipStream_t s);

hipError_t adam_multi_launch(int count, float *const *p, float *const *g, float *const *m, float *const *v,
                             const int64_t *n, const float *lr, const float *wd, float b1, float b2, float eps,
                             int step, const int32_t *step_dev, int zero_grad, hipStream_t s);

constexpr int kMlpMaxBlocks = 512;
constexpr int kMlpNarrowMaxBlocks = 512;
bool mlp_supported(int in, int h, int nh, int out);
int mlp_num_params(int in, int h, int nh, int out);
size_t mlp_workspace_bytes(int in, int h, int nh, int out);
hipError_t mlp_dispatch(bool bwd, int in, int h, int nh, int out, int64_t N, const float *x, const float *params,
                        float *y, const float *gy, float *gx, float *gparams, double *partials, hipStream_t s);

struct Options {
    int fwd_variant = -1;
    int bwd_variant = -1;
    int mlp_variant = -1;
    int bwd_compact = 1;
    int bwd_selective_zero = 1;
    int bwd_persistent = 1;
    int bwd_fork = 1;
    int bwd_item12 = -1;
    int bwd_run_pad = 1;
    int bin_acc_kib = 0;
    int bin_batch_mib = 1536;
    int tiled = -1;
    int tiled_lc_fwd = -1;
    int bwd_brick = -1;
    int bwd_brick_lo = -1;
    int bwd_brick_hi = -1;
    int bwd_brick_fork = 2;
    int bwd_brick_span = 0;
    int bwd_ext_fork = 1;
    int coord_variant = -1;
    int fwd_direct = -1;
    int triplane_layout = -1;
};
const Options &opt();
void options_snapshot();
void options_resolve_item12(int value);

__device__ __forceinline__ float relu_keep_nan(float z) { return __builtin_elementwise_maximum(z, 0.0f); }

}
```

shacira_amd/hip_ops.py:

```python
import ctypes
import functools
import threading
import weakref

import numpy as np
import torch

from . import _lib

_DTYPES = {torch.float32: _lib.F32, torch.float16: _lib.F16, torch.float64: _lib.F64}


def _stream(t):
    return ctypes.c_void_p(torch.cuda.current_stream(t.device).cuda_stream)


def _ptr(t):
    return ctypes.c_void_p(t.data_ptr()) if t is not None else None


def _ptr_array(tensors):
    return (ctypes.c_void_p * len(tensors))(*[t.data_ptr() for t in tensors])


@functools.lru_cache(maxsize=64)
def _res_array(resolutions):
    return (ctypes.c_int32 * len(resolutions))(*resolutions)


_warned = set()


def warn_unfused(what, why):
    key = (what, why)
    if key not in _warned:
        _warned.add(key)
        import warnings
        warnings.warn(f"shacira_amd: {what} runs as torch ops, not as the fused HIP kernel ({why})", RuntimeWarning,
                      stacklevel=3)


def _need_gpu(*tensors):
    for t in tensors:
        if t is not None and not t.is_cuda:
            raise RuntimeError("shacira_amd: operands must be on the MI355X (HIP) device; there is no CPU fallback")


def _check_coords(dim, coords):
    if coords.dim() != 2 or coords.shape[1] != dim or not coords.is_contiguous():
        raise RuntimeError(f"shacira_amd: coords must be a contiguous [N, {dim}] tensor for the {dim}-D operator, got "
                           f"{tuple(coords.shape)}")


def _check_float_coords(dim, coords, *others):
    _need_gpu(coords, *others)
    if coords.dtype != torch.float32:
        raise RuntimeError("expected scalar type Float for coords")
    _check_coords(dim, coords)


def _check_grad_output(grad_output, N, K):
    if grad_output.dtype != torch.float32:
        grad_output = grad_output.float()
    grad_output = grad_output.contiguous()
    _need_gpu(grad_output)
    if tuple(grad_output.shape) != (N, K):
        raise RuntimeError(f"grad_output must be [{N}, {K}], got {tuple(grad_output.shape)}")
    return grad_output


_tls = threading.local()


class _Scratch:
    __slots__ = ("buffers", "__weakref__")

    def __init__(self):
        self.buffers = {}


_all_scratch = weakref.WeakSet()
_all_scratch_lock = threading.Lock()
_SHRINK_AFTER = 64


def _workspace(device, nbytes):
    if nbytes <= 0:
        return None
    if torch.cuda.is_current_stream_capturing():
        return torch.empty((nbytes,), dtype=torch.uint8, device=device)
    scratch = getattr(_tls, "scratch", None)
    if scratch is None:
        scratch = _tls.scratch = _Scratch()
        with _all_scratch_lock:
            _all_scratch.add(scratch)
    key = (device.index, torch.cuda.current_stream(device).cuda_stream)
    entry = scratch.buffers.get(key)
    if entry is not None and entry[0].numel() >= nbytes:
        if nbytes * 4 < entry[0].numel():
            entry[1] += 1
            if entry[1] < _SHRINK_AFTER:
                return entry[0]
        else:
            entry[1] = 0
            return entry[0]
    scratch.buffers.pop(key, None)
    entry = None
    buf = torch.empty((nbytes,), dtype=torch.uint8, device=device)
    scratch.buffers[key] = [buf, 0]
    return buf


def release_workspaces(all_threads=True):
    freed = 0
    with _all_scratch_lock:
        targets = list(_all_scratch) if all_threads else [getattr(_tls, "scratch", None)]
    for sc in targets:
        if sc is None:
            continue
        for key in list(sc.buffers):
            entry = sc.buffers.pop(key, None)
            if entry is not None:
                freed += entry[0].numel()
    return freed


def retained_workspace_bytes():
    with _all_scratch_lock:
        return sum(e[0].numel() for sc in list(_all_scratch) for e in list(sc.buffers.values()))


@functools.lru_cache(maxsize=4096)
def _ws_bytes(kind, dim, N, L, F, bw, res, T, dt, epoch):
    fn = (_lib.lib().shacira_hashgrid_forward_workspace_bytes, _lib.lib().shacira_hashgrid_backward_workspace_bytes,
          _lib.lib().shacira_hashgrid_plan_bytes, _lib.lib().shacira_hashgrid_backward_planned_workspace_bytes)[kind]
    return int(fn(dim, N, L, F, bw, _res_array(res), T, dt))


def hashgrid_plan_bytes(dim, num_coords, table_rows, table_dtype, resolution, codebook_bitwidth, feature_dim):
    res = tuple(int(r) for r in resolution)
    return _ws_bytes(2, dim, int(num_coords), len(res), int(feature_dim), int(codebook_bitwidth), res, int(table_rows),
                     _DTYPES[table_dtype], _lib.options_epoch)


def hashgrid_backward_workspace_bytes(dim, num_coords, table_rows, table_dtype, resolution, codebook_bitwidth, feature_dim,
                                      planned=False):
    res = tuple(int(r) for r in resolution)
    return _ws_bytes(3 if planned else 1, dim, int(num_coords), len(res), int(feature_dim), int(codebook_bitwidth), res,
                     int(table_rows), _DTYPES[table_dtype], _lib.options_epoch)


def hashgrid_plan_buffer(dim, coords, codebook, resolution, codebook_bitwidth):
    n = hashgrid_plan_bytes(dim, coords.shape[0], codebook.shape[0], codebook.dtype, resolution, codebook_bitwidth,
                            codebook.shape[1])
    return torch.empty((n,), dtype=torch.uint8, device=codebook.device) if n > 0 else None


class _on_device:
    __slots__ = ("ctx",)

    def __init__(self, device):
        self.ctx = None if torch.cuda.current_device() == device.index else torch.cuda.device(device)

    def __enter__(self):
        if self.ctx is not None:
            self.ctx.__enter__()

    def __exit__(self, *exc):
        if self.ctx is not None:
            self.ctx.__exit__(*exc)


def _dtype_code(t):
    try:
        return _DTYPES[t.dtype]
    except KeyError:
        raise RuntimeError(f"shacira_amd: unsupported table dtype {t.dtype} (fp32, fp16 and fp64 are implemented)")


def _hashgrid_forward(dim, coords, codebook, codebook_first_idx, resolution, codebook_bitwidth, plan=None, plan_ready=False):
    _check_float_coords(dim, coords, codebook, codebook_first_idx)
    res = tuple(int(r) for r in resolution)
    N, T, F = coords.shape[0], codebook.shape[0], codebook.shape[1]
    feats = torch.empty((N, F * len(res)), dtype=codebook.dtype, device=codebook.device)
    dt = _dtype_code(codebook)
    L = _lib.lib()
    with _on_device(codebook.device):
        nbytes = _ws_bytes(0, dim, N, len(res), F, int(codebook_bitwidth), res, T, dt, _lib.options_epoch)
        ws = _workspace(codebook.device, nbytes)
        if plan is None:
            rc = L.shacira_hashgrid_forward(dim, N, len(res), F, int(codebook_bitwidth), _res_array(res),
                                            _ptr(codebook_first_idx), T, _ptr(coords), _ptr(codebook), dt, _ptr(feats),
                                            _ptr(ws), nbytes, _stream(codebook))
        else:
            _need_gpu(plan)
            rc = L.shacira_hashgrid_forward_planned(dim, N, len(res), F, int(codebook_bitwidth), _res_array(res),
                                                    _ptr(codebook_first_idx), T, _ptr(coords), _ptr(codebook), dt,
                                                    _ptr(feats), _ptr(plan), plan.numel(),
                                                    _lib.PLAN_READY if plan_ready else 0, _ptr(ws), nbytes,
                                                    _stream(codebook))
    _lib.check(rc, "hashgrid_interpolate")
    return feats


def hashgrid_backward(dim, coords, grad_output, table_rows, table_dtype, codebook_first_idx, resolution,
                      codebook_bitwidth, feature_dim, levels=None, out=None, workspace=None, flags=0, plan=None):
    _need_gpu(coords, grad_output, codebook_first_idx)
    _check_coords(dim, coords)
    res = tuple(int(r) for r in resolution)
    N, T, F = coords.shape[0], int(table_rows), int(feature_dim)
    if table_dtype not in _DTYPES:
        raise RuntimeError(f"shacira_amd: unsupported table dtype {table_dtype} (fp32, fp16 and fp64 are implemented)")
    dt = _DTYPES[table_dtype]
    if grad_output.dtype != table_dtype:
        grad_output = grad_output.to(table_dtype)
    device = grad_output.device
    if out is not None:
        if tuple(out.shape) != (T, F) or out.dtype != table_dtype or not out.is_contiguous():
            raise RuntimeError("out must be a contiguous [table_rows, feature_dim] tensor of the table dtype")
        grad_codebook = out
    else:
        if levels is not None and tuple(levels) != (0, len(res)):
            raise RuntimeError("a level range needs an existing `out` buffer (other rows are left untouched)")
        grad_codebook = torch.empty((T, F), dtype=table_dtype, device=device)
    lb, le = (0, len(res)) if levels is None else (int(levels[0]), int(levels[1]))
    L = _lib.lib()
    with _on_device(device):
        planned = plan is not None and (lb, le) == (0, len(res)) and not flags
        kind = 3 if planned and grad_output.data_ptr() % 16 == 0 else 1
        nbytes = _ws_bytes(kind, dim, N, len(res), F, int(codebook_bitwidth), res, T, dt, _lib.options_epoch)
        if workspace is not None:
            if workspace.numel() * workspace.element_size() < nbytes:
                raise RuntimeError("workspace too small")
            ws = workspace
        elif levels is not None and tuple(levels) != (0, len(res)):
            ws = torch.empty((nbytes,), dtype=torch.uint8, device=device) if nbytes else None
        else:
            ws = _workspace(device, nbytes)
        if planned:
            _need_gpu(plan)
            rc = L.shacira_hashgrid_backward_planned(dim, N, len(res), F, int(codebook_bitwidth), _res_array(res),
                                                     _ptr(codebook_first_idx), T, _ptr(coords), _ptr(grad_output), dt,
                                                     _ptr(grad_codebook), _ptr(plan), plan.numel(), _ptr(ws), nbytes,
                                                     _stream(grad_output))
        else:
            rc = L.shacira_hashgrid_backward_levels(dim, N, len(res), F, int(codebook_bitwidth), _res_array(res),
                                                    _ptr(codebook_first_idx), T, _ptr(coords), _ptr(grad_output), dt,
                                                    _ptr(grad_codebook), lb, le, int(flags), _ptr(ws), nbytes,
                                                    _stream(grad_output))
    _lib.check(rc, "hashgrid_interpolate_backward")
    return grad_codebook


def hashgrid_coords_backward(dim, coords, grad_output, codebook, codebook_first_idx, resolution, codebook_bitwidth,
                             plan=None):
    _check_float_coords(dim, coords, grad_output, codebook, codebook_first_idx)
    res = tuple(int(r) for r in resolution)
    N, T, F = coords.shape[0], codebook.shape[0], codebook.shape[1]
    dt = _dtype_code(codebook)
    codebook = codebook.contiguous()
    if grad_output.dtype != codebook.dtype:
        grad_output = grad_output.to(codebook.dtype)
    grad_output = grad_output.contiguous()
    if tuple(grad_output.shape) != (N, len(res) * F):
        raise RuntimeError(f"grad_output must be [{N}, {len(res) * F}], got {tuple(grad_output.shape)}")
    grad_coords = torch.empty((N, dim), dtype=torch.float32, device=coords.device)
    L = _lib.lib()
    with _on_device(coords.device):
        nbytes = int(L.shacira_hashgrid_coords_backward_workspace_bytes(dim, N, len(res), F, int(codebook_bitwidth),
                                                                         _res_array(res), T, dt))
        ws = _workspace(coords.device, nbytes)
        if plan is not None:
            _need_gpu(plan)
        rc = L.shacira_hashgrid_coords_backward(dim, N, len(res), F, int(codebook_bitwidth), _res_array(res),
                                                _ptr(codebook_first_idx), T, _ptr(coords), _ptr(codebook),
                                                _ptr(grad_output), dt, _ptr(grad_coords), _ptr(plan),
                                                0 if plan is None else plan.numel(), _ptr(ws), nbytes,
                                                _stream(coords))
    _lib.check(rc, "hashgrid_coords_backward")
    return grad_coords


def hashgrid_coords_backward2(dim, coords, grad_output, grad_grad_coords, codebook, codebook_first_idx, resolution,
                              codebook_bitwidth, want=(True, True, True), plan=None):
    _check_float_coords(dim, coords, grad_output, grad_grad_coords, codebook, codebook_first_idx)
    want = tuple(bool(w) for w in want)
    if len(want) != 3:
        raise RuntimeError("want must have three entries: (grad_grad_output, grad_codebook, grad_coords)")
    if not any(want):
        return None, None, None
    if codebook.dtype not in (torch.float32, torch.float16):
        raise RuntimeError(f"shacira_amd: the second-order hash-grid gradients are implemented for fp32 and fp16 tables, "
                           f"not {codebook.dtype}")
    res = tuple(int(r) for r in resolution)
    N, T, F = coords.shape[0], codebook.shape[0], codebook.shape[1]
    dt = _dtype_code(codebook)
    device = coords.device
    codebook = codebook.contiguous()
    if grad_output.dtype != codebook.dtype:
        grad_output = grad_output.to(codebook.dtype)
    grad_output = grad_output.contiguous()
    if tuple(grad_output.shape) != (N, len(res) * F):
        raise RuntimeError(f"grad_output must be [{N}, {len(res) * F}], got {tuple(grad_output.shape)}")
    v = grad_grad_coords
    if v.dtype != torch.float32:
        v = v.float()
    v = v.contiguous()
    if tuple(v.shape) != (N, dim):
        raise RuntimeError(f"grad_grad_coords must be [{N}, {dim}], got {tuple(v.shape)}")
    ggo = torch.empty((N, len(res) * F), dtype=codebook.dtype, device=device) if want[0] else None
    gcb = torch.empty((T, F), dtype=codebook.dtype, device=device) if want[1] else None
    gc = torch.empty((N, dim), dtype=torch.float32, device=device) if want[2] else None
    if N == 0 and (not want[1] or T == 0):
        return ggo, gcb, gc
    L = _lib.lib()
    with _on_device(device):
        nbytes = 0
        if want[1]:
            nbytes = int(L.shacira_hashgrid_coords_backward2_workspace_bytes(dim, N, len(res), F, int(codebook_bitwidth),
                                                                              _res_array(res), T, dt))
        ws = _workspace(device, nbytes)
        if plan is not None:
            _need_gpu(plan)
        rc = L.shacira_hashgrid_coords_backward2(dim, N, len(res), F, int(codebook_bitwidth), _res_array(res),
                                                 _ptr(codebook_first_idx), T, _ptr(coords), _ptr(codebook),
                                                 _ptr(grad_output), _ptr(v), dt, _ptr(ggo), _ptr(gcb), _ptr(gc), _ptr(plan),
                                                 0 if plan is None else plan.numel(), _ptr(ws), nbytes, _stream(coords))
    _lib.check(rc, "hashgrid_coords_backward2")
    return ggo, gcb, gc


def hashgrid_debug_corners(dim, coords, resolution, codebook_bitwidth):
    _check_float_coords(dim, coords)
    res = tuple(int(r) for r in resolution)
    N = coords.shape[0]
    rows = torch.empty((N, len(res), 1 << dim), dtype=torch.int32, device=coords.device)
    w = torch.empty((N, len(res), 1 << dim), dtype=torch.float32, device=coords.device)
    with _on_device(coords.device):
        rc = _lib.lib().shacira_hashgrid_debug_corners(dim, N, len(res), int(codebook_bitwidth), _res_array(res),
                                                       _ptr(coords), _ptr(rows), _ptr(w), _stream(coords))
    _lib.check(rc, "hashgrid_debug_corners")
    return rows, w


def backward_workspace(dim, num_coords, table_rows, table_dtype, resolution, codebook_bitwidth, feature_dim, device,
                       planned=False):
    res = tuple(int(r) for r in resolution)
    with _on_device(device):
        query = (_lib.lib().shacira_hashgrid_backward_planned_workspace_bytes if planned
                 else _lib.lib().shacira_hashgrid_backward_workspace_bytes)
        n = query(dim, int(num_coords), len(res), int(feature_dim), int(codebook_bitwidth), _res_array(res),
                  int(table_rows), _DTYPES[table_dtype])
    return torch.empty((max(n, 1),), dtype=torch.uint8, device=device)


def hashgrid_interpolate_cuda(coords, codebook, codebook_first_idx, resolution, codebook_bitwidth, plan=None,
                              plan_ready=False):
    return _hashgrid_forward(3, coords, codebook, codebook_first_idx, resolution, codebook_bitwidth, plan, plan_ready)


def hashgrid_interpolate2d_cuda(coords, codebook, codebook_first_idx, resolution, codebook_bitwidth, plan=None,
                                plan_ready=False):
    return _hashgrid_forward(2, coords, codebook, codebook_first_idx, resolution, codebook_bitwidth, plan, plan_ready)


def hashgrid_interpolate_backward_cuda(coords, grad_output, codebook, codebook_first_idx, resolution,
                                       codebook_bitwidth, feature_dim, require_grad_coords):
    return hashgrid_backward(3, coords, grad_output, codebook.shape[0], codebook.dtype, codebook_first_idx, resolution,
                             codebook_bitwidth, feature_dim)


def hashgrid_interpolate2d_backward_cuda(coords, grad_output, codebook, codebook_first_idx, resolution,
                                         codebook_bitwidth, feature_dim, require_grad_coords):
    return hashgrid_backward(2, coords, grad_output, codebook.shape[0], codebook.dtype, codebook_first_idx, resolution,
                             codebook_bitwidth, feature_dim)


def latent_decode_supported(latent_dim, feature_dim):
    return latent_dim in (1, 2, 3, 4, 8) and feature_dim in (1, 2, 4, 8) and not (latent_dim == 8 and feature_dim == 1)


def _latent_workspace(device):
    n = _lib.lib().shacira_entropy_bits_workspace_bytes(0, 1)
    return torch.empty((n,), dtype=torch.uint8, device=device)


def _check_device_scalar(t, device):
    if t.device != device or t.dtype != torch.float32 or t.numel() != 1:
        raise RuntimeError("a device-side temperature must be one fp32 value on the table's device")


def _offsets_array(offsets):
    return (ctypes.c_int64 * len(offsets))(*[int(o) for o in offsets])


def _decode_entry(name, latent, F, offsets, sga):
    T, ld = latent.shape
    args = (T, ld, F, _ptr(latent))
    if offsets is not None:
        args = (len(offsets) - 1, _offsets_array(offsets)) + args
    if sga is not None:
        uniforms, temperature, diff_sampling = sga
        if offsets is None and torch.is_tensor(temperature):
            _check_device_scalar(temperature, latent.device)
            name, temperature = name + "_tdev", _ptr(temperature)
        else:
            temperature = float(temperature)
        args += (_ptr(uniforms), temperature, int(bool(diff_sampling)))
    return getattr(_lib.lib(), "shacira_" + name), args


def _decode_forward(name, latent, offsets, sga, div, matrix, colscale, shift, clamp_weights):
    uniforms = sga[0] if sga is not None else None
    _need_gpu(latent, uniforms, div, matrix, colscale, shift)
    T, ld = latent.shape
    F = matrix.shape[-1]
    if offsets is None and sga is not None and (tuple(uniforms.shape) != (T, ld, 2) or uniforms.dtype != torch.float32
                                                or not uniforms.is_contiguous()):
        raise RuntimeError("uniforms must be a contiguous fp32 [rows, latent_dim, 2] tensor")
    out = torch.empty((T, F), dtype=torch.float32, device=latent.device)
    with _on_device(latent.device):
        fn, args = _decode_entry(name, latent, F, offsets, sga)
        rc = fn(*args, _ptr(div), _ptr(matrix), _ptr(colscale), _ptr(shift), float(clamp_weights), _ptr(out),
                _stream(latent))
    _lib.check(rc, name)
    return out


def _decode_backward(name, latent, offsets, sga, div, matrix, colscale, shift, clamp_weights, grad_decoded, need_colscale):
    _need_gpu(latent, sga[0] if sga is not None else None, grad_decoded)
    ld, F = latent.shape[1], matrix.shape[-1]
    lead = () if offsets is None else (len(offsets) - 1,)
    dev = latent.device
    g_lat = torch.empty_like(latent)
    g_mat = torch.empty(lead + (ld, F), dtype=torch.float32, device=dev)
    g_cs = torch.empty(lead + (F,), dtype=torch.float32, device=dev) if need_colscale else None
    g_sh = torch.empty(lead + (F,), dtype=torch.float32, device=dev)
    with _on_device(dev):
        ws = _latent_workspace(dev)
        fn, args = _decode_entry(name, latent, F, offsets, sga)
        rc = fn(*args, _ptr(div), _ptr(matrix), _ptr(colscale), _ptr(shift), float(clamp_weights), _ptr(grad_decoded),
                _ptr(g_lat), _ptr(g_mat), _ptr(g_cs), _ptr(g_sh), _ptr(ws), ws.numel(), _stream(latent))
    _lib.check(rc, name)
    return g_lat, g_mat, g_cs, g_sh


def latent_decode_forward(latent, div, matrix, colscale, shift, clamp_weights):
    return _decode_forward("latent_decode_forward", latent, None, None, div, matrix, colscale, shift, clamp_weights)


def latent_decode_backward(latent, div, matrix, colscale, shift, clamp_weights, grad_decoded, need_colscale):
    return _decode_backward("latent_decode_backward", latent, None, None, div, matrix, colscale, shift, clamp_weights,
                            grad_decoded, need_colscale)


def latent_decode_sga_forward(latent, uniforms, temperature, diff_sampling, div, matrix, colscale, shift, clamp_weights):
    return _decode_forward("latent_decode_sga_forward", latent, None, (uniforms, temperature, diff_sampling), div, matrix,
                           colscale, shift, clamp_weights)


def latent_decode_sga_backward(latent, uniforms, temperature, diff_sampling, div, matrix, colscale, shift, clamp_weights,
                               grad_decoded, need_colscale):
    return _decode_backward("latent_decode_sga_backward", latent, None, (uniforms, temperature, diff_sampling), div, matrix,
                            colscale, shift, clamp_weights, grad_decoded, need_colscale)


def latent_decode_levels_forward(latent, offsets, uniforms, temperature, diff_sampling, div, matrix, colscale, shift,
                                 clamp_weights):
    return _decode_forward("latent_decode_levels_forward", latent, offsets, (uniforms, temperature, diff_sampling), div,
                           matrix, colscale, shift, clamp_weights)


def latent_decode_levels_backward(latent, offsets, uniforms, temperature, diff_sampling, div, matrix, colscale, shift,
                                  clamp_weights, grad_decoded):
    return _decode_backward("latent_decode_levels_backward", latent, offsets, (uniforms, temperature, diff_sampling), div,
                            matrix, colscale, shift, clamp_weights, grad_decoded, colscale is not None)


LATENT_ACTIVATIONS = {"none": 0, "sigmoid": 1, "tanh": 2, "relu": 3, "sine": 4}


def _widths_array(widths):
    return (ctypes.c_int32 * len(widths))(*[int(w) for w in widths])


def latent_mlp_supported(widths):
    return len(widths) >= 2 and bool(_lib.lib().shacira_latent_mlp_supported(len(widths) - 1, _widths_array(widths)))


def _check_mlp_operands(latent, uniforms, div, params, widths):
    _need_gpu(latent, uniforms, div, params)
# ... 660 lines not shown
```

Measured before the change: 1.473 billion.

## Fuse sort count and partition kernels, compute per-block counts in partition pass

Merges the separate histogram-count kernel into the partition kernel, so each tile computes its own coarse-bin histogram and per-block counts in one pass and writes records into its own region of the intermediate buffer. The local sort kernel then reconstructs bin totals and per-block totals from the per-tile count and offset tables, stored in 16-bit form when they fit. This removes one kernel launch and one full read of the coordinates, at the cost of extra column reductions in the local kernel. Forward workspace sizing also stops reserving plan bytes when the caller supplies the plan.

Measured after the change: 1.491 billion, median of 6. 1.01x the previous value.

```diff
diff --git a/shacira_amd/csrc/api.hip b/shacira_amd/csrc/api.hip
--- a/shacira_amd/csrc/api.hip
+++ b/shacira_amd/csrc/api.hip
@@ -157,9 +157,9 @@
     if (num_coords < 0) return SHACIRA_EINVAL;
     if (num_coords == 0) return 0;
     if (!codebook_first_idx || !coords || !codebook || !feats) return SHACIRA_EINVAL;
-    const size_t need = hashgrid_forward_workspace(dim, dtype, lt, num_coords);
+    const bool sorts = dtype != SHACIRA_F64 && table_rows > 0 && tiled_supported(dim, dtype, lt, num_coords);
+    const size_t need = hashgrid_forward_workspace(dim, dtype, lt, num_coords, plan != nullptr && sorts);
     if (need > 0 && (!workspace || workspace_bytes < need)) return SHACIRA_EWORKSPACE;
-    const bool sorts = dtype != SHACIRA_F64 && table_rows > 0 && tiled_supported(dim, dtype, lt, num_coords);
     if (plan != nullptr && sorts && plan_bytes < sample_plan_bytes(dim, num_coords)) return SHACIRA_EWORKSPACE;
     if ((plan_flags & ~SHACIRA_PLAN_READY) != 0 || ((plan_flags & SHACIRA_PLAN_READY) != 0 && plan == nullptr)) return SHACIRA_EINVAL;
     return (int)hashgrid_forward_dispatch(dim, dtype, lt, codebook_first_idx, coords, codebook, feats, workspace,
diff --git a/shacira_amd/csrc/hashgrid_fwd.hip b/shacira_amd/csrc/hashgrid_fwd.hip
--- a/shacira_amd/csrc/hashgrid_fwd.hip
+++ b/shacira_amd/csrc/hashgrid_fwd.hip
@@ -856,9 +856,9 @@
     return hipSuccess;
 }
 
-size_t hashgrid_forward_workspace(int dim, int dtype, const LevelTable &lt, int64_t n) {
+size_t hashgrid_forward_workspace(int dim, int dtype, const LevelTable &lt, int64_t n, bool caller_plan) {
     if (dtype == SHACIRA_F64) return 0;
-    if (tiled_supported(dim, dtype, lt, n)) return tiled_forward_workspace(dim, dtype, lt, n);
+    if (tiled_supported(dim, dtype, lt, n)) return tiled_forward_workspace(dim, dtype, lt, n, caller_plan);
     if (lt.feature_dim != 2 && lt.feature_dim != 4) return 0;
     if (use_lds_tables(dim, dtype == SHACIRA_F32 ? 4 : 2, lt, n)) return 0;
     size_t b = ((size_t)n * lt.num_lods * lt.feature_dim * (dtype == SHACIRA_F32 ? 4 : 2) + 255) / 256 * 256;
diff --git a/shacira_amd/csrc/hashgrid_tiled.hip b/shacira_amd/csrc/hashgrid_tiled.hip
--- a/shacira_amd/csrc/hashgrid_tiled.hip
+++ b/shacira_amd/csrc/hashgrid_tiled.hip
@@ -24,6 +24,7 @@
     int32_t lc;
     uint32_t coarse_shift, num_coarse;
     uint32_t ptiles, chunks_per_tile;
+    uint32_t bcnt_stride, bcnt16;
 };
 
 struct TileCtx {
@@ -31,9 +32,10 @@
     float4 *sorted4;
     uint32_t *block_start;
     uint32_t *cnt;
+    uint32_t *coff;
     float4 *inter4;
+    void *bcnt;
     uint32_t *gcursor;
-    uint32_t *cbase;
 };
 
 static inline size_t up256(size_t v) { return (v + 255) / 256 * 256; }
@@ -78,6 +80,8 @@
     tp.chunks_per_tile = (uint32_t)((chunks + kMaxSortTiles - 1) / kMaxSortTiles);
     if (tp.chunks_per_tile < 1) tp.chunks_per_tile = 1;
     tp.ptiles = (uint32_t)((chunks + tp.chunks_per_tile - 1) / tp.chunks_per_tile);
+    tp.bcnt_stride = (tp.num_blocks + 63u) / 64u * 64u;
+    tp.bcnt16 = (uint64_t)kSortTileS * tp.chunks_per_tile < 65536u ? 1u : 0u;
 }
 
 static void make_tile_plan(int dim, const LevelTable &lt, int64_t n, TilePlan &tp) {
@@ -109,18 +113,21 @@
     return off;
 }
 static size_t carve_scratch(int dim, int64_t n, void *buf, TileCtx &c) {
-    (void)dim;
+    TilePlan tp;
+    make_sort_plan(dim, n, tp);
     size_t off = 0;
     auto take = [&](size_t b) { size_t o = off; off = up256(off + b); return o; };
     const size_t o_cnt = take((size_t)kMaxSortTiles * kMaxCoarse * 4);
+    const size_t o_coff = take((size_t)kMaxSortTiles * kMaxCoarse * 4);
     const size_t o_inter = take((size_t)n * sizeof(float4));
-    const size_t o_cb = take((size_t)(kMaxCoarse + 1) * 4);
-    const size_t o_gc = take((size_t)2 * kMaxBlocksS * 4);
+    const size_t o_bc = take((size_t)tp.ptiles * tp.bcnt_stride * (tp.bcnt16 ? 2 : 4));
+    const size_t o_gc = take((size_t)kMaxBlocksS * 4);
     unsigned char *p = static_cast<unsigned char *>(buf);
     if (p) {
         c.cnt = reinterpret_cast<uint32_t *>(p + o_cnt);
+        c.coff = reinterpret_cast<uint32_t *>(p + o_coff);
         c.inter4 = reinterpret_cast<float4 *>(p + o_inter);
-        c.cbase = reinterpret_cast<uint32_t *>(p + o_cb);
+        c.bcnt = p + o_bc;
         c.gcursor = reinterpret_cast<uint32_t *>(p + o_gc);
     }
     return off;
@@ -151,83 +158,61 @@
 constexpr uint32_t kLocalCap = kLocalR * kSortThreadsS;
 
 template <int DIM>
-__global__ __launch_bounds__(kSortThreadsS) void psort_count_kernel(TilePlan tp, const float *__restrict__ coords,
-                                                                    int64_t N, uint32_t *__restrict__ cnt,
-                                                                    uint32_t *__restrict__ gcursor) {
-    __shared__ uint32_t s_hist[kMaxCoarse];
-    if (threadIdx.x < kMaxCoarse) s_hist[threadIdx.x] = 0;
-    if (blockIdx.x == 0)
-        for (uint32_t k = threadIdx.x; k < 2u * kMaxBlocksS; k += kSortThreadsS) gcursor[k] = 0u;
-    __syncthreads();
-    constexpr int U = kSortTileS / kSortThreadsS;
-    for (uint32_t ch = 0; ch < tp.chunks_per_tile; ++ch) {
-        const int64_t s0 = ((int64_t)blockIdx.x * tp.chunks_per_tile + ch) * kSortTileS;
-        if (s0 >= N) break;
-        float c[U][DIM];
-        load_chunk_coords<DIM>(coords, s0, N, c);
-#pragma unroll
-        for (int u = 0; u < U; ++u)
-            if (s0 + u * kSortThreadsS + threadIdx.x < N) atomicAdd(&s_hist[block_key<DIM>(c[u], tp) >> tp.coarse_shift], 1u);
-    }
-    __syncthreads();
-    if (threadIdx.x < kMaxCoarse) cnt[(size_t)threadIdx.x * kMaxSortTiles + blockIdx.x] = s_hist[threadIdx.x];
+__device__ __forceinline__ void store_record(float4 *__restrict__ inter4, uint32_t pos, const float (&c)[DIM], int64_t i) {
+    typedef float f32x4 __attribute__((ext_vector_type(4)));
+    const f32x4 rec = {c[0], c[1], DIM == 3 ? c[DIM - 1] : 0.0f, __uint_as_float((uint32_t)i)};
+    *reinterpret_cast<f32x4 *>(inter4 + pos) = rec;
 }
 
 template <int DIM>
 __global__ __launch_bounds__(kSortThreadsS) void psort_partition_kernel(TilePlan tp, const float *__restrict__ coords,
-                                                                        int64_t N, const uint32_t *__restrict__ cnt,
-                                                                        uint32_t *__restrict__ cbase,
+                                                                        int64_t N, uint32_t *__restrict__ cnt,
+                                                                        uint32_t *__restrict__ coff,
+                                                                        void *__restrict__ bcnt,
                                                                         uint32_t *__restrict__ gcursor,
                                                                         float4 *__restrict__ inter4) {
-    __shared__ uint32_t s_cursor[kMaxCoarse], s_tot[kMaxCoarse], s_before[kMaxCoarse];
+    __shared__ uint32_t s_hist[kMaxCoarse], s_off[kMaxCoarse], s_cursor[kMaxCoarse];
     __shared__ uint32_t s_wave[kMaxCoarse / 64];
+    __shared__ uint32_t s_blk[kMaxBlocksS];
     const uint32_t lane = threadIdx.x & 63, wave = threadIdx.x >> 6;
     constexpr int U = kSortTileS / kSortThreadsS;
     float c0[U][DIM];
     const int64_t first_s0 = (int64_t)blockIdx.x * tp.chunks_per_tile * kSortTileS;
-    load_chunk_coords<DIM>(coords, first_s0 < N ? first_s0 : 0, N, c0);
-    typedef uint32_t u32x4 __attribute__((ext_vector_type(4)));
-    constexpr int kWaves = kSortThreadsS / 64, kBinsPerWave = kMaxCoarse / kWaves;
-    const bool wide = tp.ptiles > 256u;
-#ifndef SHACIRA_SORT_RB
-#define SHACIRA_SORT_RB 8
-#endif
-    constexpr int RB = SHACIRA_SORT_RB;
-#pragma unroll 1
-    for (int g = 0; g < kBinsPerWave; g += RB) {
-        u32x4 v[RB], w[RB];
-#pragma unroll
-        for (int k = 0; k < RB; ++k) {
-            const u32x4 *row = reinterpret_cast<const u32x4 *>(cnt + (size_t)(wave * kBinsPerWave + g + k) * kMaxSortTiles);
-            v[k] = row[lane];
-            w[k] = wide ? row[64 + lane] : u32x4{0u, 0u, 0u, 0u};
-        }
-#pragma unroll
-        for (int k = 0; k < RB; ++k) {
-            uint32_t tot = 0, before = 0;
-#pragma unroll
-            for (int e = 0; e < 4; ++e) {
-                const uint32_t t0 = lane * 4u + (uint32_t)e, t1 = 256u + t0;
-                const uint32_t a = t0 < tp.ptiles ? v[k][e] : 0u, b2 = t1 < tp.ptiles ? w[k][e] : 0u;
-                tot += a + b2;
-                before += (t0 < blockIdx.x ? a : 0u) + (t1 < blockIdx.x ? b2 : 0u);
+    load_chunk_coords<DIM>(coords, first_s0, N, c0);
+    if (threadIdx.x < kMaxCoarse) s_hist[threadIdx.x] = 0u;
+    for (uint32_t k = threadIdx.x; k < tp.bcnt_stride; k += kSortThreadsS) s_blk[k] = 0u;
+    if (blockIdx.x == 0)
+        for (uint32_t k = threadIdx.x; k < (uint32_t)kMaxBlocksS; k += kSortThreadsS) gcursor[k] = 0u;
+    __syncthreads();
+    for (uint32_t ch = 1; ch < tp.chunks_per_tile; ++ch) {
+        const int64_t s0 = first_s0 + (int64_t)ch * kSortTileS;
+        if (s0 >= N) break;
+        float c[U][DIM];
+        load_chunk_coords<DIM>(coords, s0, N, c);
+#pragma unroll
+        for (int u = 0; u < U; ++u)
+            if (s0 + u * kSortThreadsS + threadIdx.x < N) {
+                const uint32_t key = block_key<DIM>(c[u], tp);
+                atomicAdd(&s_hist[key >> tp.coarse_shift], 1u);
+                atomicAdd(&s_blk[key], 1u);
             }
-#pragma unroll
-            for (int off = 32; off > 0; off >>= 1) {
-                tot += __shfl_xor(tot, off, 64);
-                before += __shfl_xor(before, off, 64);
-            }
-            if (lane == 0) {
-                s_tot[wave * kBinsPerWave + g + k] = tot;
-                s_before[wave * kBinsPerWave + g + k] = before;
-            }
-        }
+    }
+    if (tp.chunks_per_tile > 1u) __syncthreads();
+    uint32_t bin0[U], rank0[U];
+#pragma unroll
+    for (int u = 0; u < U; ++u) {
+        const bool live = first_s0 + u * kSortThreadsS + threadIdx.x < N;
+        const uint32_t key = block_key<DIM>(c0[u], tp);
+        bin0[u] = key >> tp.coarse_shift;
+        rank0[u] = live ? atomicAdd(&s_hist[bin0[u]], 1u) : 0xFFFFFFFFu;
+        if (live) atomicAdd(&s_blk[key], 1u);
     }
     __syncthreads();
     const bool owner = threadIdx.x < kMaxCoarse;
-    uint32_t tot = 0;
+    uint32_t excl = 0;
     if (owner) {
-        tot = s_tot[threadIdx.x];
+        const uint32_t tot = s_hist[threadIdx.x];
+        cnt[(size_t)threadIdx.x * kMaxSortTiles + blockIdx.x] = tot;
         uint32_t incl = tot;
 #pragma unroll
         for (int off = 1; off < 64; off <<= 1) {
@@ -235,72 +220,40 @@
             if (lane >= (uint32_t)off) incl += nbr;
         }
         if (lane == 63) s_wave[wave] = incl;
-        s_cursor[threadIdx.x] = incl - tot;
-    }
-    __syncthreads();
-    uint32_t base = 0;
+        excl = incl - tot;
+    }
+    if (tp.bcnt16) {
+        uint32_t *row = static_cast<uint32_t *>(bcnt) + (size_t)blockIdx.x * (tp.bcnt_stride / 2u);
+        for (uint32_t k = threadIdx.x; k < tp.bcnt_stride / 2u; k += kSortThreadsS) row[k] = s_blk[2u * k] | (s_blk[2u * k + 1u] << 16);
+    } else {
+        uint32_t *row = static_cast<uint32_t *>(bcnt) + (size_t)blockIdx.x * tp.bcnt_stride;
+        for (uint32_t k = threadIdx.x; k < tp.bcnt_stride; k += kSortThreadsS) row[k] = s_blk[k];
+    }
+    __syncthreads();
     if (owner) {
+        uint32_t base = excl;
         for (uint32_t wv = 0; wv < wave; ++wv) base += s_wave[wv];
-        base += s_cursor[threadIdx.x];
-        if (blockIdx.x == 0) {
-            cbase[threadIdx.x] = base;
-            if (threadIdx.x == kMaxCoarse - 1) cbase[kMaxCoarse] = base + tot;
-        }
-    }
-    __shared__ uint32_t s_over_any;
-    __shared__ uint32_t s_blk[kMaxBlocksS];
-    if (threadIdx.x == 0) s_over_any = 0u;
-    __syncthreads();
-    if (owner) {
-        s_cursor[threadIdx.x] = base + s_before[threadIdx.x];
-        if (tot > kLocalCap) s_over_any = 1u;
-        s_tot[threadIdx.x] = tot > kLocalCap ? 1u : 0u;
-    }
-    __syncthreads();
-    const bool over_any = s_over_any != 0u;
-    if (over_any) {
-        for (uint32_t k = threadIdx.x; k < tp.num_blocks; k += kSortThreadsS) s_blk[k] = 0u;
-        __syncthreads();
-    }
-    for (uint32_t ch = 0; ch < tp.chunks_per_tile; ++ch) {
+        s_off[threadIdx.x] = base;
+        s_cursor[threadIdx.x] = base;
+        coff[(size_t)threadIdx.x * kMaxSortTiles + blockIdx.x] = base;
+    }
+    __syncthreads();
+    float4 *region = inter4 + first_s0;
+    for (uint32_t ch = 1; ch < tp.chunks_per_tile; ++ch) {
         const int64_t s0 = first_s0 + (int64_t)ch * kSortTileS;
         if (s0 >= N) break;
         float c[U][DIM];
-        if (ch == 0) {
-#pragma unroll
-            for (int u = 0; u < U; ++u)
-#pragma unroll
-                for (int a = 0; a < DIM; ++a) c[u][a] = c0[u][a];
-        } else {
-            load_chunk_coords<DIM>(coords, s0, N, c);
-        }
-        uint32_t pos[U];
+        load_chunk_coords<DIM>(coords, s0, N, c);
 #pragma unroll
         for (int u = 0; u < U; ++u) {
             const int64_t i = s0 + u * kSortThreadsS + threadIdx.x;
-            const uint32_t key = block_key<DIM>(c[u], tp);
-            pos[u] = (i < N) ? atomicAdd(&s_cursor[key >> tp.coarse_shift], 1u) : 0xFFFFFFFFu;
-            if (over_any && i < N && s_tot[key >> tp.coarse_shift]) atomicAdd(&s_blk[key], 1u);
-        }
-#pragma unroll
-        for (int u = 0; u < U; ++u) {
-            const int64_t i = s0 + u * kSortThreadsS + threadIdx.x;
-            if (pos[u] != 0xFFFFFFFFu) {
-                typedef float f32x4 __attribute__((ext_vector_type(4)));
-                const f32x4 rec = {c[u][0], c[u][1], DIM == 3 ? c[u][DIM - 1] : 0.0f, __uint_as_float((uint32_t)i)};
-#ifdef SHACIRA_SORT_NT
-                __builtin_nontemporal_store(rec, reinterpret_cast<f32x4 *>(inter4 + pos[u]));
-#else
-                *reinterpret_cast<f32x4 *>(inter4 + pos[u]) = rec;
-#endif
-            }
-        }
-    }
-    if (over_any) {
-        __syncthreads();
-        uint32_t *gcount = gcursor + kMaxBlocksS;
-        for (uint32_t k = threadIdx.x; k < tp.num_blocks; k += kSortThreadsS)
-            if (s_blk[k]) atomicAdd(&gcount[k], s_blk[k]);
+            if (i < N) store_record<DIM>(region, atomicAdd(&s_cursor[block_key<DIM>(c[u], tp) >> tp.coarse_shift], 1u), c[u], i);
+        }
+    }
+#pragma unroll
+    for (int u = 0; u < U; ++u) {
+        const int64_t i = first_s0 + u * kSortThreadsS + threadIdx.x;
+        if (rank0[u] != 0xFFFFFFFFu) store_record<DIM>(region, s_off[bin0[u]] + rank0[u], c0[u], i);
     }
 }
 
@@ -319,47 +272,136 @@
     return live ? atomicAdd(&counters[j], 1u) : 0u;
 }
 
+__device__ __forceinline__ void bin_totals(const TilePlan &tp, const uint32_t *__restrict__ cnt, uint32_t *s_tot) {
+    typedef uint32_t u32x4 __attribute__((ext_vector_type(4)));
+    constexpr uint32_t kWaves = kSortThreadsS / 64;
+    constexpr int RB = 8;
+    const uint32_t lane = threadIdx.x & 63, wave = threadIdx.x >> 6;
+    const bool wide = tp.ptiles > 256u;
+#pragma unroll 1
+    for (uint32_t r0 = wave; r0 < (uint32_t)kMaxCoarse; r0 += kWaves * RB) {
+        u32x4 v[RB], w[RB];
+#pragma unroll
+        for (int k = 0; k < RB; ++k) {
+            const u32x4 *row = reinterpret_cast<const u32x4 *>(cnt + (size_t)(r0 + (uint32_t)k * kWaves) * kMaxSortTiles);
+            v[k] = row[lane];
+            w[k] = wide ? row[64 + lane] : u32x4{0u, 0u, 0u, 0u};
+        }
+#pragma unroll
+        for (int k = 0; k < RB; ++k) {
+            uint32_t tot = 0;
+#pragma unroll
+            for (int e = 0; e < 4; ++e) {
+                const uint32_t t0 = lane * 4u + (uint32_t)e, t1 = 256u + t0;
+                tot += (t0 < tp.ptiles ? v[k][e] : 0u) + (t1 < tp.ptiles ? w[k][e] : 0u);
+            }
+#pragma unroll
+            for (int off = 32; off > 0; off >>= 1) tot += __shfl_xor(tot, off, 64);
+            if (lane == 0) s_tot[r0 + (uint32_t)k * kWaves] = tot;
+        }
+    }
+}
+
+__device__ __forceinline__ uint32_t bcnt_at(const void *__restrict__ bcnt, const TilePlan &tp, uint32_t tile, uint32_t block) {
+    const size_t i = (size_t)tile * tp.bcnt_stride + block;
+    return tp.bcnt16 ? (uint32_t)static_cast<const uint16_t *>(bcnt)[i] : static_cast<const uint32_t *>(bcnt)[i];
+}
+
 template <int DIM>
 __global__ __launch_bounds__(kSortThreadsS) void psort_local_kernel(TilePlan tp, const float4 *__restrict__ inter4,
-                                                                    const uint32_t *__restrict__ cbase,
-                                                                    const uint32_t *__restrict__ gcount,
+                                                                    const uint32_t *__restrict__ cnt,
+                                                                    const uint32_t *__restrict__ coff,
+                                                                    const void *__restrict__ bcnt,
                                                                     uint32_t *__restrict__ gcursor,
                                                                     float4 *__restrict__ sorted4,
                                                                     uint32_t *__restrict__ block_start,
                                                                     uint32_t *__restrict__ header, uint32_t n) {
     constexpr int kBpc = kMaxBlocksS / kMaxCoarse;
     constexpr int R = kLocalR;
-    uint32_t bin, lo, hi, c_lo, c_hi;
+    constexpr uint32_t kScanWaves = kMaxSortTiles / 64;
+    __shared__ uint32_t s_pre[kMaxSortTiles];
+    __shared__ uint32_t s_src[kMaxSortTiles];
+    __shared__ uint32_t s_wrow[kScanWaves], s_wcol[kScanWaves];
+    const uint32_t lane = threadIdx.x & 63, wave = threadIdx.x >> 6;
     const bool first = blockIdx.x < tp.num_coarse;
+    uint32_t bin = blockIdx.x, p0 = 0;
+    if (!first) {
+        p0 = (blockIdx.x - tp.num_coarse) * kLocalCap;
+        if (p0 >= n) return;
+        __shared__ uint32_t s_rowtot[kMaxCoarse], s_wtot4[kMaxCoarse / 64], s_le;
+        if (threadIdx.x == 0) s_le = 0u;
+        bin_totals(tp, cnt, s_rowtot);
+        __syncthreads();
+        uint32_t incl = 0, tot = 0;
+        if (threadIdx.x < kMaxCoarse) {
+            tot = s_rowtot[threadIdx.x];
+            incl = tot;
+#pragma unroll
+            for (int off = 1; off < 64; off <<= 1) {
+                const uint32_t nbr = __shfl_up(incl, off, 64);
+                if (lane >= (uint32_t)off) incl += nbr;
+            }
+            if (lane == 63) s_wtot4[wave] = incl;
+        }
+        __syncthreads();
+        if (threadIdx.x < kMaxCoarse) {
+            uint32_t base = incl - tot;
+            for (uint32_t wv = 0; wv < wave; ++wv) base += s_wtot4[wv];
+            const uint64_t le = __ballot(threadIdx.x < tp.num_coarse && base <= p0);
+            if (lane == 0 && le) atomicAdd(&s_le, (uint32_t)__popcll(le));
+        }
+        __syncthreads();
+        bin = s_le - 1u;
+    }
+    const uint32_t t = threadIdx.x & (kMaxSortTiles - 1);
+    uint32_t rowv = cnt[(size_t)bin * kMaxSortTiles + t], colv = coff[(size_t)bin * kMaxSortTiles + t];
+    if (threadIdx.x >= (uint32_t)kMaxSortTiles || t >= tp.ptiles) rowv = colv = 0u;
+    uint32_t incl = rowv, csum = colv;
+#pragma unroll
+    for (int off = 1; off < 64; off <<= 1) {
+        const uint32_t nbr = __shfl_up(incl, off, 64);
+        if (lane >= (uint32_t)off) incl += nbr;
+    }
+#pragma unroll
+    for (int off = 32; off > 0; off >>= 1) csum += __shfl_xor(csum, off, 64);
+    if (wave < kScanWaves && lane == 63) {
+        s_wrow[wave] = incl;
+        s_wcol[wave] = csum;
+    }
+    __syncthreads();
+    uint32_t lo = 0, tot = 0, pre = incl - rowv;
+    for (uint32_t wv = 0; wv < kScanWaves; ++wv) {
+        const uint32_t rw = s_wrow[wv];
+        if (wv < wave) pre += rw;
+        tot += rw;
+        lo += s_wcol[wv];
+    }
+    const uint32_t hi = lo + tot;
+    if (threadIdx.x < (uint32_t)kMaxSortTiles) {
+        s_pre[t] = pre;
+        s_src[t] = t * tp.chunks_per_tile * (uint32_t)kSortTileS + colv - pre;
+    }
+    uint32_t c_lo, c_hi;
     if (first) {
-        bin = blockIdx.x;
-        lo = cbase[bin];
-        hi = cbase[bin + 1];
         c_lo = lo;
         c_hi = (lo + kLocalCap < hi) ? lo + kLocalCap : hi;
     } else {
-        const uint32_t p0 = (blockIdx.x - tp.num_coarse) * kLocalCap;
-        if (p0 >= n) return;
-        __shared__ uint32_t s_le;
-        if (threadIdx.x == 0) s_le = 0u;
-        __syncthreads();
-        uint32_t c = (threadIdx.x < tp.num_coarse && cbase[threadIdx.x] <= p0) ? 1u : 0u;
-        if (threadIdx.x < kMaxCoarse) {
-#pragma unroll
-            for (int off = 32; off > 0; off >>= 1) c += __shfl_xor(c, off, 64);
-            if ((threadIdx.x & 63u) == 0u && c) atomicAdd(&s_le, c);
-        }
-        __syncthreads();
-        bin = s_le - 1u;
-        lo = cbase[bin];
-        hi = cbase[bin + 1];
         c_lo = (lo + kLocalCap > p0) ? lo + kLocalCap : p0;
         c_hi = (p0 + kLocalCap < hi) ? p0 + kLocalCap : hi;
         if (c_lo >= c_hi) return;
     }
+    __syncthreads();
+    auto fetch = [&](uint32_t p) {
+        const uint32_t k = p - lo;
+        uint32_t tl = 0;
+#pragma unroll
+        for (uint32_t step = kMaxSortTiles / 2; step > 0; step >>= 1)
+            if (s_pre[tl + step] <= k) tl += step;
+        const uint32_t a = s_src[tl] + k;
+        return inter4[a < n ? a : n - 1u];
+    };
     const uint32_t key0 = bin << tp.coarse_shift;
     const uint32_t bpc = 1u << tp.coarse_shift;
-    const uint32_t lane = threadIdx.x & 63;
     auto key_of = [&](const float4 &r) {
         float cc[DIM];
         cc[0] = r.x;
@@ -372,7 +414,7 @@
         header[1] = tp.num_blocks;
         header[2] = n;
     }
-    if (first && hi - lo <= kLocalCap) {
+    if (first && tot <= kLocalCap) {
 #ifndef SHACIRA_SORT_SUB
 #define SHACIRA_SORT_SUB 2
 #endif
@@ -402,7 +444,7 @@
 #pragma unroll
         for (int u = 0; u < R; ++u) {
             const uint32_t p = lo + (uint32_t)u * kSortThreadsS + threadIdx.x;
-            r[u] = inter4[p < hi ? p : (hi > 0u ? hi - 1u : 0u)];
+            r[u] = fetch(p < hi ? p : (hi > lo ? hi - 1u : lo));
         }
 #pragma unroll
         for (int u = 0; u < R; ++u) {
@@ -413,28 +455,28 @@
         __syncthreads();
         {
             constexpr int KPT = (kKeys + kSortThreadsS - 1) / kSortThreadsS;
-            uint32_t cnt[KPT], sum = 0;
+            uint32_t kc[KPT], sum = 0;
 #pragma unroll
             for (int q = 0; q < KPT; ++q) {
                 const uint32_t k = threadIdx.x * KPT + q;
-                cnt[q] = k < (uint32_t)kKeys ? s_tot8[k] : 0u;
-                sum += cnt[q];
+                kc[q] = k < (uint32_t)kKeys ? s_tot8[k] : 0u;
+                sum += kc[q];
             }
-            uint32_t incl = sum;
+            uint32_t kincl = sum;
 #pragma unroll
             for (int off = 1; off < 64; off <<= 1) {
-                const uint32_t nbr = __shfl_up(incl, off, 64);
-                if (lane >= (uint32_t)off) incl += nbr;
+                const uint32_t nbr = __shfl_up(kincl, off, 64);
+                if (lane >= (uint32_t)off) kincl += nbr;
             }
-            if (lane == 63) s_wtot[threadIdx.x >> 6] = incl;
+            if (lane == 63) s_wtot[wave] = kincl;
             __syncthreads();
-            uint32_t run = incl - sum;
-            for (uint32_t w = 0; w < (threadIdx.x >> 6); ++w) run += s_wtot[w];
+            uint32_t run = kincl - sum;
+            for (uint32_t w = 0; w < wave; ++w) run += s_wtot[w];
 #pragma unroll
             for (int q = 0; q < KPT; ++q) {
                 const uint32_t k = threadIdx.x * KPT + q;
                 if (k < (uint32_t)kKeys) s_off8[k] = run;
-                run += cnt[q];
+                run += kc[q];
             }
         }
         __syncthreads();
@@ -445,16 +487,35 @@
             if (lo + (uint32_t)u * kSortThreadsS + threadIdx.x < hi) sorted4[lo + s_off8[j[u]] + rk[u]] = r[u];
         return;
     }
-    __shared__ uint32_t s_off[kBpc + 1], s_cnt[kBpc], s_base[kBpc];
+    __shared__ uint32_t s_off[kBpc + 1], s_btot[kBpc], s_cnt[kBpc], s_base[kBpc];
+    if (threadIdx.x < kBpc) {
+        s_btot[threadIdx.x] = 0u;
+        s_cnt[threadIdx.x] = 0u;
+    }
+    __syncthreads();
+    {
+        const uint32_t b = threadIdx.x & (kBpc - 1u);
+        const bool col = b < bpc && key0 + b < tp.num_blocks;
+        const uint32_t blk = col ? key0 + b : tp.num_blocks - 1u;
+        uint32_t sum = 0;
+        for (uint32_t t0 = 0; t0 < tp.ptiles; t0 += kSortThreadsS / kBpc) {
+            const uint32_t tl = t0 + threadIdx.x / kBpc;
+            const uint32_t v = bcnt_at(bcnt, tp, tl < tp.ptiles ? tl : tp.ptiles - 1u, blk);
+            sum += (col && tl < tp.ptiles) ? v : 0u;
+        }
+        sum += __shfl_xor(sum, 16, 64);
+        sum += __shfl_xor(sum, 32, 64);
+        if (lane < (uint32_t)kBpc && sum) atomicAdd(&s_btot[b], sum);
+    }
+    __syncthreads();
     if (threadIdx.x == 0) {
         uint32_t run = 0;
         for (uint32_t b = 0; b < bpc; ++b) {
             s_off[b] = run;
-            run += (key0 + b < tp.num_blocks) ? gcount[key0 + b] : 0u;
+            run += s_btot[b];
         }
         s_off[bpc] = run;
     }
-    if (threadIdx.x < kBpc) s_cnt[threadIdx.x] = 0;
     __syncthreads();
     if (first) {
         if (threadIdx.x < bpc && key0 + threadIdx.x < tp.num_blocks) block_start[key0 + threadIdx.x] = lo + s_off[threadIdx.x];
@@ -465,7 +526,7 @@
 #pragma unroll
     for (int u = 0; u < R; ++u) {
         const uint32_t p = c_lo + (uint32_t)u * kSortThreadsS + threadIdx.x;
-        r[u] = inter4[p < c_hi ? p : c_hi - 1u];
+        r[u] = fetch(p < c_hi ? p : c_hi - 1u);
     }
 #pragma unroll
     for (int u = 0; u < R; ++u) {
@@ -518,14 +579,11 @@
     carve_plan(n, plan, c);
     carve_scratch(dim, n, scratch, c);
     const uint32_t chunks = tp.num_coarse + (uint32_t)((n + kLocalCap - 1) / kLocalCap);
-    uint32_t *gcount = c.gcursor + kMaxBlocksS;
-#define SHACIRA_SORT_LAUNCHES(D)                                                                                          \
-    hipLaunchKernelGGL(psort_count_kernel<D>, dim3(tp.ptiles), dim3(kSortThreadsS), 0, s, tp, coords, n, c.cnt, c.gcursor);  \
-    SHACIRA_CHECK_LAUNCH();                                                                                                  \
-    hipLaunchKernelGGL(psort_partition_kernel<D>, dim3(tp.ptiles), dim3(kSortThreadsS), 0, s, tp, coords, n, c.cnt, c.cbase, \
-                       c.gcursor, c.inter4);                                                                                 \
-    SHACIRA_CHECK_LAUNCH();                                                                                                  \
-    hipLaunchKernelGGL(psort_local_kernel<D>, dim3(chunks), dim3(kSortThreadsS), 0, s, tp, c.inter4, c.cbase, gcount,        \
+#define SHACIRA_SORT_LAUNCHES(D)                                                                                            \
+    hipLaunchKernelGGL(psort_partition_kernel<D>, dim3(tp.ptiles), dim3(kSortThreadsS), 0, s, tp, coords, n, c.cnt, c.coff, c.bcnt, \
+                       c.gcursor, c.inter4);                                                                                   \
+    SHACIRA_CHECK_LAUNCH();                                                                                                    \
+    hipLaunchKernelGGL(psort_local_kernel<D>, dim3(chunks), dim3(kSortThreadsS), 0, s, tp, c.inter4, c.cnt, c.coff, c.bcnt,   \
                        c.gcursor, c.sorted4, c.block_start, c.header, (uint32_t)n);
     if (dim == 3) {
         SHACIRA_SORT_LAUNCHES(3)
@@ -557,8 +615,8 @@
     for (int a = 0; a < 3; ++a) out.nb[a] = tp.nb[a];
 }
 
-size_t tiled_forward_workspace(int dim, int dtype, const LevelTable &lt, int64_t n) {
-    return staged_bytes(dtype, lt, n) + scratch_bytes_of(dim, n) + plan_bytes_of(n);
+size_t tiled_forward_workspace(int dim, int dtype, const LevelTable &lt, int64_t n, bool caller_plan) {
+    return staged_bytes(dtype, lt, n) + scratch_bytes_of(dim, n) + (caller_plan ? 0 : plan_bytes_of(n));
 }
 
 hipError_t tiled_forward(int dim, int dtype, const LevelTable &lt, const int32_t *first_idx, const float *coords,
diff --git a/shacira_amd/csrc/internal.h b/shacira_amd/csrc/internal.h
--- a/shacira_amd/csrc/internal.h
+++ b/shacira_amd/csrc/internal.h
@@ -21,7 +21,7 @@
     }
 };
 
-size_t hashgrid_forward_workspace(int dim, int dtype, const LevelTable &lt, int64_t n);
+size_t hashgrid_forward_workspace(int dim, int dtype, const LevelTable &lt, int64_t n, bool caller_plan = false);
 hipError_t hashgrid_forward_dispatch(int dim, int dtype, const LevelTable &lt, const int32_t *first_idx,
                                      const float *coords, const void *table, void *feats, void *workspace, int64_t n,
                                      hipStream_t s, void *plan = nullptr, bool plan_ready = false);
@@ -31,7 +31,7 @@
 hipError_t hashgrid_forward_rows(int dim, int dtype, const LevelTable &lt, const int32_t *first_idx, const float *sorted4,
                                  const void *table, const void *staged, void *feats, int64_t n, int lc, hipStream_t s);
 bool tiled_supported(int dim, int dtype, const LevelTable &lt, int64_t n);
-size_t tiled_forward_workspace(int dim, int dtype, const LevelTable &lt, int64_t n);
+size_t tiled_forward_workspace(int dim, int dtype, const LevelTable &lt, int64_t n, bool caller_plan = false);
 hipError_t tiled_forward(int dim, int dtype, const LevelTable &lt, const int32_t *first_idx, const float *coords,
                          const void *table, void *feats, void *workspace, int64_t n, hipStream_t s, void *plan = nullptr,
                          bool plan_ready = false);
diff --git a/shacira_amd/hip_ops.py b/shacira_amd/hip_ops.py
--- a/shacira_amd/hip_ops.py
+++ b/shacira_amd/hip_ops.py
@@ -187,6 +187,8 @@
     L = _lib.lib()
     with _on_device(codebook.device):
         nbytes = _ws_bytes(0, dim, N, len(res), F, int(codebook_bitwidth), res, T, dt, _lib.options_epoch)
+        if plan is not None:
+            nbytes -= _ws_bytes(2, dim, N, len(res), F, int(codebook_bitwidth), res, T, dt, _lib.options_epoch)
         ws = _workspace(codebook.device, nbytes)
         if plan is None:
             rc = L.shacira_hashgrid_forward(dim, N, len(res), F, int(codebook_bitwidth), _res_array(res),
```
